# anthonyhu/tumblr-emotions

Measured on AMD Instinct MI355X. Metric: training samples/sec (224x224 img + 32-tok text, batch 256), higher is better.
Workload: dtype f32; 1 GPU; joint train step (fwd+bwd+all-reduce+Adam): Inception-v1 224x224x3 + 300-d embedding + LSTM-512, T=32, V=10000, 15 classes, batch 256 per GPU, reference freeze (<=Mixed_5b conv weights frozen, all BN betas trainable), dropout 0.8, BN train mode; global_batch=256, per_gpu_batch=256, parallelism=dp1, launch=eager

## Files before the change

### include/ds_kernels.h

```cpp
#ifndef DS_KERNELS_H
#define DS_KERNELS_H

#include <stddef.h>
#include <stdint.h>

#ifdef __cplusplus
extern "C" {
#endif

#define DS_OK 0
#define DS_ERR_ARG (-1)
#define DS_ERR_LAUNCH (-2)
#define DS_ERR_WORKSPACE (-3)

#define DS_DTYPE_F32 0
#define DS_DTYPE_BF16 1

#define DS_EPI_BIAS 1
#define DS_EPI_RELU 2
#define DS_EPI_ACCUM 4
#define DS_EPI_STATS 8
#define DS_EPI_MASK 16
#define DS_EPI_BNSUMS 32
#define DS_EPI_BN_RELU 64
// ... 203 lines not shown
int ds_conv_plan_enable_pool3(ds_conv_layer_plan *plan, uint8_t *argmax);
int ds_conv_plan_enable_bn_relu(ds_conv_layer_plan *plan);
int ds_conv_plan_finalize_tickets(const ds_conv_layer_plan *plan);
int ds_conv_prepare_weights(const ds_conv_layer_plan *plan, const float *w_hwio, void *w_prepared, float *wscale,
                            void *stream);
int ds_conv_run(const ds_conv_layer_plan *plan, const void *x, const void *w, float *z, const ds_conv_io *io, void *stream);

size_t ds_conv_wgrad_workspace(const ds_conv_desc *d);
int ds_conv_wgrad(const ds_conv_desc *d, const float *x, const float *dz, int32_t lddz, float *dw,
                  void *ws, size_t ws_bytes, void *stream);

int ds_bn_finalize(const float *stats, int32_t P, int64_t count, int32_t C, const float *beta, const float *pivot,
                   float eps, float decay, float *mean, float *rstd, float *shift, float *moving_mean,
                   float *moving_var, void *stream);

int ds_bn_finalize_centered(const float *stats, int32_t P, int64_t count, int32_t C, const float *beta, const float *pivot,
                            float eps, float decay, float *mean, float *rstd, float *shift, float *moving_mean,
                            float *moving_var, float *mean_c, float *shift_c, void *stream);
typedef struct ds_bn_finalize_job {
    const float *stats;
    int32_t P, C;
    int64_t count;
    const float *beta;
    const float *pivot;
    float *mean, *rstd, *shift;
    float *moving_mean, *moving_var;
} ds_bn_finalize_job;
int ds_bn_finalize_multi(const ds_bn_finalize_job *jobs, int32_t njobs, float eps, float decay, void *stream);

int ds_bn_finalize_apply_relu(const float *stats, int32_t P, int64_t count, int32_t C, const float *beta, const float *pivot,
                              float eps, float decay, float *mean, float *rstd, float *shift, float *moving_mean,
                              float *moving_var, const float *z, int64_t M, const struct ds_segments *dst, uint32_t *ticket,
                              void *stream);

typedef struct ds_segments {
    int32_t nseg;
    int32_t c_begin[4];
    int32_t c_end[4];
    int32_t ld[4];
    void *ptr[4];
    int32_t dtype[4];
    float *amax[4];
    const float *ptr2[4];
} ds_segments;
int ds_bn_apply_relu(const float *z, int64_t M, int32_t C, const float *rstd, const float *shift,
                     const ds_segments *dst, void *stream);
int ds_bn_apply_relu_z16(const void *z16, int64_t M, int32_t C, const float *rstd, const float *shift,
                         const ds_segments *dst, void *stream);
int ds_bn_infer_prepare(const float *beta, const float *moving_mean, const float *moving_var, float eps,
                        int32_t C, float *rstd, float *shift, void *stream);
typedef struct ds_bn_infer_job {
    const float *beta, *moving_mean, *moving_var;
    int32_t C;
    float *rstd, *shift;
} ds_bn_infer_job;
int ds_bn_infer_prepare_multi(const ds_bn_infer_job *jobs, int32_t njobs, float eps, void *stream);

int ds_bn_bwd_partials(int64_t M, int32_t C);
int ds_bn_bwd_reduce(const void *z, int32_t ldz, int32_t z_dtype, const ds_segments *dy, int64_t M, int32_t C,
                     const float *mean, const float *rstd, const float *shift, float *partials, void *stream);
int ds_bn_bwd_finalize(const float *partials, int32_t P, int64_t M, int32_t C, float *dbeta, float *coef,
                       void *stream);
typedef struct ds_bn_sum_segments {
    int32_t nseg;
    int32_t c_begin[4], c_end[4];
    int32_t P[4];
    int32_t kind[4];
    const float *s[4];
    const float *q[4];
    int32_t P2[4];
    const float *s2[4];
    const float *q2[4];
} ds_bn_sum_segments;
int ds_bn_bwd_finalize_segs(const ds_bn_sum_segments *sg, int64_t M, int32_t C, const float *beta, float *dbeta,
                            float *coef, void *stream);
int ds_bn_bwd_finalize_multi(const ds_bn_sum_segments *sg, int64_t M, int32_t C, const float *const *beta,
                             float *const *dbeta, float *coef, void *stream);
int ds_bn_bwd_finalize_apply(const ds_bn_sum_segments *sg, const float *beta, float *dbeta, const float *const *beta_v,
                             float *const *dbeta_v, float *coef, const float *z, int32_t ldz, const ds_segments *dy, int64_t M,
                             int32_t C, const float *mean, const float *rstd, const float *shift, void *dz, int32_t dz_dtype,
                             int32_t lddz, float *amax, uint32_t *ticket, void *stream);
int ds_bn_bwd_apply(const float *z, int32_t ldz, const ds_segments *dy, int64_t M, int32_t C, const float *mean,
                    const float *rstd, const float *shift, const float *coef, float *dz, float *amax, void *stream);
int ds_bn_infer_bwd_apply(const float *z, int32_t ldz, const ds_segments *dy, int64_t M, int32_t C, const float *rstd,
                          const float *shift, float *dz, void *stream);
int ds_bn_infer_bwd_partials(int64_t M, int32_t C);
int ds_bn_infer_bwd_apply_sums(const float *z, int32_t ldz, const ds_segments *dy, int64_t M, int32_t C, const float *rstd,
                               const float *shift, float *dz, float *partials, void *stream);
typedef struct ds_bn_sum_job {
    const float *partials;
    int32_t P, C;
    float *dbeta;
} ds_bn_sum_job;
int ds_bn_dbeta_reduce_multi(const ds_bn_sum_job *jobs, int32_t njobs, void *stream);
int ds_bn_bwd_apply_bf16(const float *z, int32_t ldz, const ds_segments *dy, int64_t M, int32_t C, const float *mean,
                         const float *rstd, const float *shift, const float *coef, void *dz16, int32_t lddz, float *amax,
                         void *stream);

int ds_bn_bwd_apply_z16(const void *z16, int32_t ldz, const ds_segments *dy, int64_t M, int32_t C, const float *mean,
                        const float *rstd, const float *shift, const float *coef, void *dz16, int32_t lddz, float *amax,
                        void *stream);

int ds_maxpool_fwd(const void *x, void *y, uint8_t *argmax, int32_t N, int32_t H, int32_t W, int32_t C,
                   int32_t k, int32_t stride, int32_t pad_t, int32_t pad_l, int32_t OH, int32_t OW,
                   int32_t act_dtype, void *stream);
int ds_maxpool_bn_relu_fwd(const float *z, const float *rstd, const float *shift, void *y, uint8_t *argmax,
                           int32_t N, int32_t H, int32_t W, int32_t C, int32_t k, int32_t stride, int32_t pad_t,
                           int32_t pad_l, int32_t OH, int32_t OW, int32_t y_dtype, float *amax, void *stream);
int ds_bn_pool_bwd_partials(int32_t N, int32_t OH, int32_t OW, int32_t C);
int ds_bn_pool_bwd_reduce(const float *z, const float *dpool, const uint8_t *argmax, int32_t N, int32_t H, int32_t W,
                          int32_t C, int32_t pad_t, int32_t pad_l, int32_t OH, int32_t OW, const float *mean,
                          const float *rstd, const float *shift, float *partials, void *stream);
int ds_bn_pool_bwd_apply(const float *z, const float *dpool, const uint8_t *argmax, int32_t N, int32_t H, int32_t W,
                         int32_t C, int32_t pad_t, int32_t pad_l, int32_t OH, int32_t OW, const float *mean,
                         const float *rstd, const float *shift, const float *coef, float *dz, void *stream);
int ds_bn_pool_infer_bwd_apply(const float *z, const float *dpool, const uint8_t *argmax, int32_t N, int32_t H, int32_t W,
                               int32_t C, int32_t pad_t, int32_t pad_l, int32_t OH, int32_t OW, const float *rstd,
                               const float *shift, float *dz, void *stream);
int ds_bn_pool_infer_bwd_apply_sums(const float *z, const float *dpool, const uint8_t *argmax, int32_t N, int32_t H, int32_t W,
                                    int32_t C, int32_t pad_t, int32_t pad_l, int32_t OH, int32_t OW, const float *rstd,
                                    const float *shift, float *dz, float *partials, void *stream);
int ds_maxpool_bwd(const float *dy, const uint8_t *argmax, float *dx, int32_t accumulate, int32_t N,
                   int32_t H, int32_t W, int32_t C, int32_t k, int32_t stride, int32_t pad_t, int32_t pad_l,
                   int32_t OH, int32_t OW, void *stream);

int ds_maxpool3_bwd_sums_partials(int32_t N, int32_t W, int32_t C);
int ds_maxpool3_bwd_sums(const float *dy, const uint8_t *argmax, float *dx, int32_t accumulate, const void *y,
                         int32_t y_dtype, int32_t N, int32_t H, int32_t W, int32_t C, float *partials, void *stream);

int ds_maxpool3_bwd_dy16(const void *dy16, const uint8_t *argmax, float *dx, int32_t accumulate, const void *y, int32_t y_dtype,
                         int32_t N, int32_t H, int32_t W, int32_t C, float *partials, void *stream);

int ds_avgpool_dropout_fwd(const float *x, int32_t N, int32_t HW, int32_t C, float keep, uint64_t seed,
                           const uint64_t *seed_dev, const float *mask_in, float *mask_out, float *out,
                           void *stream);
int ds_avgpool_dropout_bwd(const float *dout, const float *mask, int32_t N, int32_t HW, int32_t C,
                           float keep, float *dx, void *stream);

int ds_gather_rows(const float *table, const int64_t *ids, float *out, int32_t B, int32_t T, int32_t D,
                   int64_t table_rows, int32_t time_major, void *stream);

int ds_token_dot(const float *dx, const float *x, const int64_t *seq_len, float *out, int32_t B, int32_t T, int32_t D,
                 void *stream);

int ds_embedding_grad(const float *dx, const int64_t *ids, float *dtable, int32_t B, int32_t T, int32_t D,
                      int64_t table_rows, int32_t time_major, void *stream);

int ds_lstm_cell_fwd(float *gates, const float *rec_slabs, int32_t nslabs, int64_t slab_stride,
                     const float *c_prev, const float *h_prev, const int64_t *seq_len, int32_t t, int32_t B,
                     int32_t H, float forget_bias, float *c_out, float *h_out, void *stream);
int ds_lstm_cell_bwd(const float *acts, const float *c_t, const float *c_prev, const float *dh,
                     const float *dh_slabs, int32_t nslabs, int64_t slab_stride, const float *dc,
                     const int64_t *seq_len, int32_t t, int32_t B, int32_t H, float *dgates, float *dc_prev,
                     float *dh_carry, void *stream);

int ds_seq_sort_desc(const int64_t *seq_len, int32_t B, int32_t T, int32_t *perm, int64_t *len_sorted, void *stream);
int ds_permute_rows(const void *src, int64_t lds, void *dst, int64_t ldd, const int32_t *perm, int32_t rows, int32_t cols,
                    int32_t elem_bytes, int32_t gather, void *stream);
#define DS_LSTM_SKIP_MASKED 256
int ds_lstm_seq_supported(int32_t B, int32_t H);
size_t ds_lstm_seq_workspace(int32_t B, int32_t H);
int ds_lstm_seq_fwd(float *gates, const float *wh, int32_t ldw, float *h, float *c, const int64_t *seq_len, int32_t T,
                    int32_t B, int32_t H, float forget_bias, int32_t rows, void *ws, size_t ws_bytes, void *stream);
int ds_lstm_seq_bwd(const float *acts, const float *wh, int32_t ldw, const float *c, const float *dh_last,
                    int32_t ld_dh, const int64_t *seq_len, int32_t T, int32_t B, int32_t H, float *dgates, int32_t rows,
                    void *ws, size_t ws_bytes, void *stream);
int ds_lstm_seq_status(void *ws, int32_t B);
#ifdef DS_TUNING
int ds_debug_lstm_seq_set_profile(void *buf);
int ds_debug_lstm_seq_set_profile_bwd(void *buf);
#endif

int ds_softmax_ce(const float *logits, const int64_t *labels, int32_t B, int32_t C, float grad_scale,
                  const float *grad_scale_dev, float *loss, float *dlogits, void *stream);

int ds_adam_tf(float *theta, const float *g, float *m, float *v, int64_t n, int64_t n_wd, float wd,
               float grad_scale, float lr_t, const float *lr_t_dev, float beta1, float beta2, float eps,
               void *stream);

int ds_sumsq(const float *x, int64_t n, float *scratch, float *out, void *stream);
int ds_colsum(const float *x, int64_t M, int32_t C, int32_t ld, float *scratch, float *out, void *stream);
int ds_slab_epilogue(const float *slabs, int32_t splits, int64_t slab_stride, int32_t lds, int64_t M, int32_t N, float *out,
                     int32_t ldo, const float *bias, const float *mask, int32_t ldmask, int32_t flags, void *stream);
int ds_copy2d(const float *src, int32_t lds, float *dst, int32_t ldd, int64_t rows, int32_t cols,
              void *stream);
int ds_pad_channels(const float *src, int32_t cs, float *dst, int32_t cd, int64_t pixels, void *stream);
int ds_fill(float *dst, int64_t n, float value, void *stream);

typedef struct ds_preprocess_desc {
    int64_t offset;
    int32_t height, width;
    float scale_y, scale_x;
} ds_preprocess_desc;
int ds_preprocess_eval(const uint8_t *bytes, int64_t nbytes, const ds_preprocess_desc *desc, int32_t batch, const float *lut,
                       float *out, int32_t out_h, int32_t out_w, void *stream);

#define DS_PREPROCESS_FLIP 1u
#define DS_PREPROCESS_SATURATION_FIRST 2u
// ... 115 lines not shown
```

### tumblr_emotions_amd/_lib.py

```python
import ctypes as C
import os

_HERE = os.path.dirname(os.path.abspath(__file__))
LIB_PATH = os.environ.get("DS_LIB") or os.path.join(_HERE, "libds_kernels.so")

def tuning_env(name, default=None):
    return os.environ.get(name, default) if os.environ.get("DS_LIB") else default


DS_EPI_BIAS, DS_EPI_RELU, DS_EPI_ACCUM, DS_EPI_STATS, DS_EPI_MASK, DS_EPI_BNSUMS = 1, 2, 4, 8, 16, 32
DS_EPI_BN_RELU = 64
DS_DTYPE_F32, DS_DTYPE_BF16 = 0, 1
DS_FP8_E4M3, DS_FP8_E5M2 = 0, 1
DS_CONV_FWD, DS_CONV_DGRAD = 0, 1
DS_LSTM_SKIP_MASKED = 256
DS_ARITH_F32, DS_ARITH_BF16, DS_ARITH_FP8, DS_ARITH_F32X3 = 0, 1, 2, 3
DS_FAM_IGEMM, DS_FAM_WINO2, DS_FAM_WINO4, DS_FAM_STEM, DS_FAM_BF16D, DS_FAM_FP8D, DS_FAM_F32X3, DS_FAM_WINO4H, DS_FAM_STEM_POOL = range(9)
DS_FAM_STEM_DGRAD = 9
DS_PLAN_NO_WINO, DS_PLAN_NO_WINO4, DS_PLAN_NO_STEM_DIRECT, DS_PLAN_NO_BF16_DIRECT, DS_PLAN_ACT16, DS_PLAN_PACKED_RGB = 1, 2, 4, 8, 16, 32
DS_PLAN_FP8_EVERYWHERE, DS_PLAN_FP8_WIDE_RULE, DS_PLAN_NO_WINO4H, DS_PLAN_STEM_POOL = 64, 128, 256, 512
DS_PLAN_NO_SPLITK = 1024
DS_PREPROCESS_FLIP, DS_PREPROCESS_SATURATION_FIRST = 1, 2
DS_JPEG_UNSUPPORTED, DS_JPEG_MORE = 1, 2
DS_JPEG_444, DS_JPEG_422, DS_JPEG_420, DS_JPEG_GREY = 0, 1, 2, 3
# ... 112 lines not shown
_SS = C.POINTER(SumSegments)
_LP = C.POINTER(LayerPlanStruct)
_IO = C.POINTER(ConvIO)

SIGNATURES = {
    "ds_version": (C.c_int, []),
    "ds_last_error": (C.c_char_p, []),
    "ds_conv_igemm_partials": (C.c_int, [_CD]),
    "ds_conv_igemm_bnsums_supported": (C.c_int, [_CD]),
    "ds_conv_igemm_norm_supported": (C.c_int, [_CD]),
    "ds_conv_igemm_bnb_supported": (C.c_int, [_CD]),
    "ds_conv_igemm_pool3_supported": (C.c_int, [_CD]),
    "ds_conv_igemm_finalize_tickets": (C.c_int, [_CD]),
    "ds_conv_igemm": (C.c_int, [_CD, _P, _P, _P, _P, _P, _P, _P, _P]),
    "ds_weights_bf16_bytes": (C.c_size_t, [_i32, _i32, _i32, _i32]),
    "ds_weights_to_bf16": (C.c_int, [_P, _P, _i32, _i32, _i32, _i32, _P]),
    "ds_conv_bf16_supported": (C.c_int, [_CD]),
    "ds_conv_bf16_partials": (C.c_int, [_CD]),
    "ds_conv_bf16": (C.c_int, [_CD, _P, _P, _P, _P, _P, _P, _P]),
    "ds_weights_f32x3_bytes": (C.c_size_t, [_i32, _i32, _i32, _i32]),
    "ds_weights_to_f32x3": (C.c_int, [_P, _P, _i32, _i32, _i32, _i32, _P]),
    "ds_conv_f32x3_supported": (C.c_int, [_CD]),
    "ds_conv_f32x3_partials": (C.c_int, [_CD]),
    "ds_conv_f32x3": (C.c_int, [_CD, _P, _P, _P, _P, _P, _P, _P]),
    "ds_absmax": (C.c_int, [_P, _i64, _i32, _P, _P]),
    "ds_weights_fp8_bytes": (C.c_size_t, [_i32, _i32, _i32, _i32]),
    "ds_weights_to_fp8": (C.c_int, [_P, _P, _P, _i32, _i32, _i32, _i32, _P]),
    "ds_conv_fp8_supported": (C.c_int, [_CD]),
    "ds_conv_fp8_partials": (C.c_int, [_CD]),
    "ds_conv_fp8": (C.c_int, [_CD, _P, _P, _i32, _P, _P, _P, _P, _P, _P, _P]),
    "ds_conv_stem_partials": (C.c_int, [_i32, _i32, _i32]),
    "ds_conv_stem_bf16_partials": (C.c_int, [_i32, _i32, _i32]),
    "ds_conv_stem": (C.c_int, [_P, _P, _P, _P, _P, _i32, _i32, _i32, _i32, _i32, _i32, _P]),
    "ds_conv_stem_bf16": (C.c_int, [_P, _P, _P, _P, _P, _i32, _i32, _i32, _i32, _i32, _i32, _P]),
    "ds_conv_stem_pool_supported": (C.c_int, [_i32, _i32]),
    "ds_conv_stem_pool_partials": (C.c_int, [_i32, _i32, _i32]),
    "ds_conv_stem_pool": (C.c_int, [_P, _P, _P, _P, _P, _i32, _i32, _i32, _i32, _i32, _i32, _P]),
    "ds_conv_stem_pool_bf16": (C.c_int, [_P, _P, _P, _P, _P, _i32, _i32, _i32, _i32, _i32, _i32, _P]),
    "ds_conv_stem_dgrad_supported": (C.c_int, [_i32, _i32]),
    "ds_conv_stem_dgrad": (C.c_int, [_P, _P, _P, _i32, _i32, _i32, _i32, _i32, _P]),
    "ds_wino_transform_weights": (C.c_int, [_P, _P, _i32, _i32, _i32, _P]),
    "ds_conv_wino_partials": (C.c_int, [_i32, _i32, _i32]),
    "ds_conv_wino": (C.c_int, [_P, _P, _P, _P, _P, _P, _i32, _i32, _i32, _i32, _i32, _i32, _i32, _i32, _P]),
    "ds_conv_wino4_supported": (C.c_int, [_i32, _i32, _i32, _i32]),
    "ds_conv_wino4_prefer": (C.c_int, [_i32, _i32, _i32, _i32, _i32]),
    "ds_wino4_transform_weights": (C.c_int, [_P, _P, _i32, _i32, _i32, _P]),
    "ds_conv_wino4_partials": (C.c_int, [_i32, _i32, _i32]),
    "ds_conv_wino4_splitk_choose": (C.c_int, [_i32, _i32, _i32, _i32, _i32]),
    "ds_conv_wino4_splitk_partials": (C.c_int, [_i32, _i32, _i32]),
    "ds_conv_wino4_splitk_workspace": (C.c_size_t, [_i32, _i32, _i32, _i32, _i32]),
    "ds_conv_wino4_splitk": (C.c_int, [_P, _P, _P, _P, _P, _P, _i32, _i32, _i32, _i32, _i32, _i32, _i32, _i32, _i32, _i32, _P, C.c_size_t, _P]),
    "ds_conv_wino4": (C.c_int, [_P, _P, _P, _P, _P, _P, _i32, _i32, _i32, _i32, _i32, _i32, _i32, _i32, _P]),
    "ds_conv_wino4_bf16x2": (C.c_int, [_P, _P, _P, _P, _P, _P, _i32, _i32, _i32, _i32, _i32, _i32, _i32, _i32, _i32, _P]),
    "ds_conv_wino4_bf16x2_x16": (C.c_int, [_P, _P, _P, _P, _P, _P, _i32, _i32, _i32, _i32, _i32, _i32, _i32, _i32, _i32, _P]),
    "ds_wino4_transform_weights_bf16x2": (C.c_int, [_P, _P, _i32, _i32, _i32, _P]),
    "ds_conv_plan": (C.c_int, [_LP, _i32, _i32, C.c_uint32] + [_i32] * 10),
    "ds_conv_plan_set_flags": (C.c_int, [_LP, _i32]),
    "ds_conv_plan_enable_bnsums": (C.c_int, [_LP, _i32]),
    "ds_conv_plan_norm_supported": (C.c_int, [_LP]),
    "ds_conv_plan_bnb_supported": (C.c_int, [_LP]),
    "ds_conv_plan_enable_pool3": (C.c_int, [_LP, C.c_void_p]),
    "ds_conv_plan_enable_bn_relu": (C.c_int, [_LP]),
    "ds_conv_plan_finalize_tickets": (C.c_int, [_LP]),
    "ds_conv_prepare_weights": (C.c_int, [_LP, _P, _P, _P, _P]),
    "ds_conv_run": (C.c_int, [_LP, _P, _P, _P, _IO, _P]),
    "ds_conv_wgrad_workspace": (C.c_size_t, [_CD]),
    "ds_conv_wgrad": (C.c_int, [_CD, _P, _P, _i32, _P, _P, C.c_size_t, _P]),
    "ds_bn_finalize": (C.c_int, [_P, _i32, _i64, _i32, _P, _P, _f32, _f32, _P, _P, _P, _P, _P, _P]),
    "ds_bn_finalize_centered": (C.c_int, [_P, _i32, _i64, _i32, _P, _P, _f32, _f32, _P, _P, _P, _P, _P, _P, _P, _P]),
    "ds_bn_apply_relu": (C.c_int, [_P, _i64, _i32, _P, _P, _SG, _P]),
    "ds_bn_apply_relu_z16": (C.c_int, [_P, _i64, _i32, _P, _P, _SG, _P]),
    "ds_bn_bwd_apply_z16": (C.c_int, [_P, _i32, _SG, _i64, _i32, _P, _P, _P, _P, _P, _i32, _P, _P]),
    "ds_bn_infer_prepare": (C.c_int, [_P, _P, _P, _f32, _i32, _P, _P, _P]),
    "ds_bn_infer_prepare_multi": (C.c_int, [_P, _i32, _f32, _P]),
    "ds_bn_bwd_partials": (C.c_int, [_i64, _i32]),
    "ds_bn_bwd_reduce": (C.c_int, [_P, _i32, _i32, _SG, _i64, _i32, _P, _P, _P, _P, _P]),
    "ds_bn_bwd_finalize_segs": (C.c_int, [_SS, _i64, _i32, _P, _P, _P, _P]),
    "ds_bn_bwd_finalize": (C.c_int, [_P, _i32, _i64, _i32, _P, _P, _P]),
    "ds_bn_bwd_finalize_multi": (C.c_int, [_SS, _i64, _i32, _P, _P, _P, _P]),
    "ds_bn_finalize_multi": (C.c_int, [_P, _i32, _f32, _f32, _P]),
    "ds_bn_finalize_apply_relu": (C.c_int, [_P, _i32, _i64, _i32, _P, _P, _f32, _f32, _P, _P, _P, _P, _P, _P, _i64, _SG, _P, _P]),
    "ds_bn_bwd_finalize_apply": (C.c_int, [_SS, _P, _P, _P, _P, _P, _P, _i32, _SG, _i64, _i32, _P, _P, _P, _P, _i32, _i32, _P, _P, _P]),
    "ds_bn_bwd_apply": (C.c_int, [_P, _i32, _SG, _i64, _i32, _P, _P, _P, _P, _P, _P, _P]),
    "ds_bn_infer_bwd_apply": (C.c_int, [_P, _i32, _SG, _i64, _i32, _P, _P, _P, _P]),
    "ds_bn_infer_bwd_partials": (C.c_int, [_i64, _i32]),
    "ds_bn_infer_bwd_apply_sums": (C.c_int, [_P, _i32, _SG, _i64, _i32, _P, _P, _P, _P, _P]),
    "ds_bn_dbeta_reduce_multi": (C.c_int, [_P, _i32, _P]),
    "ds_bn_bwd_apply_bf16": (C.c_int, [_P, _i32, _SG, _i64, _i32, _P, _P, _P, _P, _P, _i32, _P, _P]),
    "ds_maxpool_fwd": (C.c_int, [_P, _P, _P] + [_i32] * 11 + [_P]),
    "ds_maxpool_bn_relu_fwd": (C.c_int, [_P, _P, _P, _P, _P] + [_i32] * 11 + [_P, _P]),
    "ds_bn_pool_bwd_partials": (C.c_int, [_i32, _i32, _i32, _i32]),
    "ds_bn_pool_bwd_reduce": (C.c_int, [_P, _P, _P] + [_i32] * 8 + [_P, _P, _P, _P, _P]),
    "ds_bn_pool_bwd_apply": (C.c_int, [_P, _P, _P] + [_i32] * 8 + [_P, _P, _P, _P, _P, _P]),
    "ds_bn_pool_infer_bwd_apply": (C.c_int, [_P, _P, _P] + [_i32] * 8 + [_P, _P, _P, _P]),
    "ds_bn_pool_infer_bwd_apply_sums": (C.c_int, [_P, _P, _P] + [_i32] * 8 + [_P, _P, _P, _P, _P]),
    "ds_maxpool_bwd": (C.c_int, [_P, _P, _P] + [_i32] * 11 + [_P]),
    "ds_maxpool3_bwd_sums_partials": (C.c_int, [_i32, _i32, _i32]),
    "ds_maxpool3_bwd_sums": (C.c_int, [_P, _P, _P, _i32, _P, _i32, _i32, _i32, _i32, _i32, _P, _P]),
    "ds_maxpool3_bwd_dy16": (C.c_int, [_P, _P, _P, _i32, _P, _i32, _i32, _i32, _i32, _i32, _P, _P]),
    "ds_avgpool_dropout_fwd": (C.c_int, [_P, _i32, _i32, _i32, _f32, _u64, _P, _P, _P, _P, _P]),
    "ds_avgpool_dropout_bwd": (C.c_int, [_P, _P, _i32, _i32, _i32, _f32, _P, _P]),
    "ds_gather_rows": (C.c_int, [_P, _P, _P, _i32, _i32, _i32, _i64, _i32, _P]),
    "ds_token_dot": (C.c_int, [_P, _P, _P, _P, _i32, _i32, _i32, _P]),
    "ds_embedding_grad": (C.c_int, [_P, _P, _P, _i32, _i32, _i32, _i64, _i32, _P]),
    "ds_lstm_cell_fwd": (C.c_int, [_P, _P, _i32, _i64, _P, _P, _P, _i32, _i32, _i32, _f32, _P, _P, _P]),
    "ds_lstm_cell_bwd": (C.c_int, [_P, _P, _P, _P, _P, _i32, _i64, _P, _P, _i32, _i32, _i32, _P, _P, _P, _P]),
    "ds_seq_sort_desc": (C.c_int, [_P, _i32, _i32, _P, _P, _P]),
    "ds_permute_rows": (C.c_int, [_P, _i64, _P, _i64, _P, _i32, _i32, _i32, _i32, _P]),
    "ds_lstm_seq_supported": (C.c_int, [_i32, _i32]),
    "ds_lstm_seq_workspace": (C.c_size_t, [_i32, _i32]),
    "ds_lstm_seq_fwd": (C.c_int, [_P, _P, _i32, _P, _P, _P, _i32, _i32, _i32, _f32, _i32, _P, C.c_size_t, _P]),
    "ds_lstm_seq_bwd": (C.c_int, [_P, _P, _i32, _P, _P, _i32, _P, _i32, _i32, _i32, _P, _i32, _P, C.c_size_t, _P]),
    "ds_lstm_seq_status": (C.c_int, [_P, _i32]),
    "ds_softmax_ce": (C.c_int, [_P, _P, _i32, _i32, _f32, _P, _P, _P, _P]),
    "ds_adam_tf": (C.c_int, [_P, _P, _P, _P, _i64, _i64, _f32, _f32, _f32, _P, _f32, _f32, _f32, _P]),
    "ds_sumsq": (C.c_int, [_P, _i64, _P, _P, _P]),
    "ds_colsum": (C.c_int, [_P, _i64, _i32, _i32, _P, _P, _P]),
    "ds_slab_epilogue": (C.c_int, [_P, _i32, _i64, _i32, _i64, _i32, _P, _i32, _P, _P, _i32, _i32, _P]),
    "ds_copy2d": (C.c_int, [_P, _i32, _P, _i32, _i64, _i32, _P]),
    "ds_pad_channels": (C.c_int, [_P, _i32, _P, _i32, _i64, _P]),
    "ds_fill": (C.c_int, [_P, _i64, _f32, _P]),
    "ds_preprocess_eval": (C.c_int, [_P, _i64, _P, _i32, _P, _P, _i32, _i32, _P]),
    "ds_preprocess_train": (C.c_int, [_P, _i64, _P, _i32, _P, _P, _i32, _i32, _P]),
    "ds_jpeg_probe": (C.c_int, [_P, _i64, C.POINTER(JpegInfo)]),
    "ds_jpeg_entropy_decode": (C.c_int, [_P, _i64, C.POINTER(JpegInfo), _P, _i64]),
    "ds_jpeg_reconstruct_host": (C.c_int, [_P, _i64, _P, _i32, _P, _i64]),
    "ds_jpeg_reconstruct": (C.c_int, [_P, _i64, _P, _i32, _P, _i64, _P, _i64, _P]),
    "ds_example_parse": (C.c_int, [_P, _i64, _P, _i32, C.POINTER(ExampleFields)]),
    "ds_jpeg_record_decode": (C.c_int, [_P, _i64, _P, _i32, C.POINTER(ExampleFields), C.POINTER(JpegInfo), _P, _i64,
                                        C.POINTER(_i32)]),
    "ds_jpeg_scan": (C.c_int, [_P, _i64, C.POINTER(JpegInfo), C.POINTER(JpegScanInfo), _P, _i64]),
    "ds_jpeg_record_scan": (C.c_int, [_P, _i64, _P, _i32, C.POINTER(ExampleFields), C.POINTER(JpegInfo), C.POINTER(JpegScanInfo),
                                      _P, _i64, C.POINTER(_i32)]),
    "ds_jpeg_restart_transcode": (C.c_int, [_P, _i64, _i32, _P, _i64, C.POINTER(_i64)]),
    "ds_jpeg_entropy_decode_segments_host": (C.c_int, [_P, _i64, _P, _i32, _P, _i64, _P, _i64, _P]),
    "ds_jpeg_entropy_decode_device": (C.c_int, [_P, _i64, _P, _i32, _P, _i64, _P, _i64, _P, _P]),
    "ds_ragged_gather": (C.c_int, [_P, _i64, _P, _i64, _P, _i32, _P, _i64, _P]),
    "ds_ragged_gather_host": (C.c_int, [_P, _i64, _P, _i64, _P, _i32, _P, _i64]),
}

_lib = None


DEBUG_SIGNATURES = {
    "ds_debug_conv_set_tile": (C.c_int, [C.c_int, C.c_int]),
    "ds_debug_conv_set_path": (C.c_int, [C.c_int]),
    "ds_debug_conv_set_wide": (C.c_int, [C.c_int]),
    "ds_debug_conv_wino_allow_ablation": (C.c_int, [C.c_int]),
    "ds_debug_conv_wino4_set_nb": (C.c_int, [C.c_int]),
    "ds_debug_conv_bf16_set_max_nb": (C.c_int, [C.c_int]),
    "ds_debug_lstm_seq_set_profile": (C.c_int, [_P]),
    "ds_debug_lstm_seq_set_profile_bwd": (C.c_int, [_P]),
}
TUNING_LIB_PATH = os.path.join(_HERE, "libds_kernels_tuning.so")
_tuning = None


def _bind(lib, table):
    for name, (res, args) in table.items():
        fn = getattr(lib, name)
        fn.restype = res
        fn.argtypes = args


def load_tuning():
    global _tuning
    if _tuning is None:
        if not os.path.exists(TUNING_LIB_PATH):
            raise RuntimeError("tumblr_emotions_amd: %s not found -- `make -C tumblr_emotions_amd/csrc` builds it" % TUNING_LIB_PATH)
        lib = C.CDLL(TUNING_LIB_PATH)
        _bind(lib, SIGNATURES)
        _bind(lib, DEBUG_SIGNATURES)
        _tuning = lib
    return _tuning


# ... 37 lines not shown
```

### tumblr_emotions_amd/csrc/bn.hip

```cpp
#include <stdlib.h>
#include "ds_common.h"

namespace {

struct SegDev {
    int nseg;
    int c_begin[4], c_end[4], ld[4];
    float *ptr[4];
    int dtype[4];
    float *amax[4];
    const float *ptr2[4];
};

SegDev to_dev(const ds_segments *s) {
    SegDev o;
    o.nseg = s->nseg;
    for (int i = 0; i < 4; ++i) {
        o.c_begin[i] = s->c_begin[i];
        o.c_end[i] = s->c_end[i];
        o.ld[i] = s->ld[i];
        o.ptr[i] = (float *)s->ptr[i];
        o.dtype[i] = s->dtype[i];
        o.amax[i] = s->amax[i];
        o.ptr2[i] = s->ptr2[i];
// ... 319 lines not shown
    s = wave_sum_f64(s);
    q = wave_sum_f64(q);
    if (lane == 0) {
        red[0][wave] = s;
        red[1][wave] = q;
    }
    __syncthreads();
    if (threadIdx.x == 0) {
        s = ((red[0][0] + red[0][1]) + red[0][2]) + red[0][3];
        q = ((red[1][0] + red[1][1]) + red[1][2]) + red[1][3];
        dbeta[c] = (float)s;
        if (coef) {
            coef[c] = (float)(s * inv_count);
            coef[C + c] = (float)(q * inv_count);
        }
    }
}

struct SumSegDev {
    int nseg;
    int c_begin[4], c_end[4], P[4], kind[4];
    const float *s[4], *q[4];
    int P2[4];
    const float *s2[4], *q2[4];
    const float *beta[4];
    float *dbeta[4];
};

template <bool COH = false>
__device__ __forceinline__ void bwd_finalize_segs_channel(const SumSegDev &sg, double inv_count, int C, float *coef, int c) {
    __shared__ double red[2][4];
    const int lane = threadIdx.x & 63, wave = threadIdx.x >> 6;
    int P = 0, kind = 0, P2 = 0;
    const float *sp = nullptr, *qp = nullptr, *beta = nullptr, *sp2 = nullptr, *qp2 = nullptr;
    float *dbeta = nullptr;
#pragma unroll
    for (int i = 0; i < 4; ++i)
        if (i < sg.nseg && c >= sg.c_begin[i] && c < sg.c_end[i]) {
            P = sg.P[i];
            kind = sg.kind[i];
            sp = sg.s[i] + (int64_t)(c - sg.c_begin[i]) * P;
            qp = sg.q[i] + (int64_t)(c - sg.c_begin[i]) * P;
            P2 = sg.P2[i];
            if (P2 > 0) {
                sp2 = sg.s2[i] + (int64_t)(c - sg.c_begin[i]) * P2;
                qp2 = sg.q2[i] + (int64_t)(c - sg.c_begin[i]) * P2;
            }
            beta = sg.beta[i] ? sg.beta[i] + (c - sg.c_begin[i]) : nullptr;
            dbeta = sg.dbeta[i] ? sg.dbeta[i] + (c - sg.c_begin[i]) : nullptr;
        }
    double s = 0.0, q = 0.0;
    for (int p = threadIdx.x; p < P; p += 256) {
        s += (double)sp[p];
        q += (double)qp[p];
    }
    for (int p = threadIdx.x; p < P2; p += 256) {
        s += (double)sp2[p];
        q += (double)qp2[p];
    }
    s = wave_sum_f64(s);
    q = wave_sum_f64(q);
    if (lane == 0) {
        red[0][wave] = s;
        red[1][wave] = q;
    }
    __syncthreads();
    if (threadIdx.x == 0) {
        s = ((red[0][0] + red[0][1]) + red[0][2]) + red[0][3];
        q = ((red[1][0] + red[1][1]) + red[1][2]) + red[1][3];
        if (kind == 1) q -= (double)*beta * s;
        if (dbeta) *dbeta = (float)s;
        st_res<COH>(coef + c, (float)(s * inv_count));
        st_res<COH>(coef + C + c, (float)(q * inv_count));
    }
}

__global__ __launch_bounds__(256) void bn_bwd_finalize_segs_kernel(SumSegDev sg, double inv_count, int C, float *coef) {
    bwd_finalize_segs_channel(sg, inv_count, C, coef, (int)blockIdx.x);
}

template <bool OUT16, bool COH = false, bool ADD2 = false, bool Z16 = false>
__device__ __forceinline__ void bwd_apply_body(int bid, const float *z, int ldz, const SegDev &dy, int64_t M, int C,
                                               const float *mean, const float *rstd, const float *shift,
                                               const float *coef, float *dz, float *amax, int drow, int lddz) {
    const int C4 = C >> 2;
    const int t0 = bid * 256 + threadIdx.x;
    const int row0 = t0 / C4, c = (t0 - row0 * C4) * 4;
    const float4 r4 = *reinterpret_cast<const float4 *>(rstd + c), s4 = *reinterpret_cast<const float4 *>(shift + c);
    const float4 m4 = *reinterpret_cast<const float4 *>(mean + c);
    const float4 k14 = ld_res4<COH>(coef + c), k24 = ld_res4<COH>(coef + C + c);
    const float rr[4] = {r4.x, r4.y, r4.z, r4.w}, ss[4] = {s4.x, s4.y, s4.z, s4.w}, mm[4] = {m4.x, m4.y, m4.z, m4.w};
    const float a1[4] = {k14.x, k14.y, k14.z, k14.w}, a2[4] = {k24.x, k24.y, k24.z, k24.w};
    int sgi = 0;
#pragma unroll
    for (int i = 1; i < 4; ++i)
        if (i < dy.nseg && c >= dy.c_begin[i] && c < dy.c_end[i]) sgi = i;
    const float *const dyp = dy.ptr[sgi] + (c - dy.c_begin[sgi]);
    const int64_t dyld = dy.ld[sgi];
    const float *const dyp2 = (ADD2 && dy.ptr2[sgi]) ? dy.ptr2[sgi] + (c - dy.c_begin[sgi]) : nullptr;
    float am = 0.f;
    constexpr int NR = DS_BN_ROWS;
    for (int64_t row = row0; row < M; row += NR * (int64_t)drow) {
        int64_t rws[NR];
        bool ok[NR];
#pragma unroll
        for (int u = 0; u < NR; ++u) {
            ok[u] = row + u * (int64_t)drow < M;
            rws[u] = ok[u] ? row + u * (int64_t)drow : row;
        }
        float4 zv[NR], dv[NR];
#pragma unroll
        for (int u = 0; u < NR; ++u) {
            if constexpr (Z16) zv[u] = ldz4<__bf16>(reinterpret_cast<const __bf16 *>(z) + rws[u] * ldz + c);
            else zv[u] = ds::ld_stream4(z + rws[u] * ldz + c);
            dv[u] = ds::ld_stream4(dyp + rws[u] * dyld);
        }
        if (ADD2 && dyp2) {
#pragma unroll
            for (int u = 0; u < NR; ++u) {
                const float4 e = ds::ld_stream4(dyp2 + rws[u] * dyld);
                dv[u].x += e.x; dv[u].y += e.y; dv[u].z += e.z; dv[u].w += e.w;
            }
        }
#pragma unroll
        for (int u = 0; u < NR; ++u) {
            if (u > 0 && !ok[u]) break;
            const float zz[4] = {zv[u].x, zv[u].y, zv[u].z, zv[u].w}, dd[4] = {dv[u].x, dv[u].y, dv[u].z, dv[u].w};
            float o[4];
#pragma unroll
            for (int j = 0; j < 4; ++j) o[j] = ds::bn_bwd_dz(zz[j], dd[j], rr[j], ss[j], mm[j], a1[j], a2[j]);
            if (OUT16) {
                const f32x4_t ov = {o[0], o[1], o[2], o[3]};
                *reinterpret_cast<bf16x4_t *>(reinterpret_cast<__bf16 *>(dz) + rws[u] * lddz + c) = __builtin_convertvector(ov, bf16x4_t);
            } else {
                *reinterpret_cast<float4 *>(dz + rws[u] * ldz + c) = make_float4(o[0], o[1], o[2], o[3]);
            }
            am = fmaxf(am, fmaxf(fmaxf(fabsf(o[0]), fabsf(o[1])), fmaxf(fabsf(o[2]), fabsf(o[3]))));
        }
    }
    if (amax) {
#pragma unroll
        for (int o = 32; o > 0; o >>= 1) am = fmaxf(am, __shfl_xor(am, o));
        if ((threadIdx.x & 63) == 0) ds::atomic_max_nonneg(amax, am);
    }
}

template <bool OUT16, bool ADD2 = false, bool Z16 = false>
__global__ __launch_bounds__(256) void bn_bwd_apply_kernel(const float *z, int ldz, SegDev dy, int64_t M, int C,
                                                           const float *mean, const float *rstd, const float *shift,
                                                           const float *coef, float *dz, float *amax, int drow, int lddz) {
    bwd_apply_body<OUT16, false, ADD2, Z16>((int)blockIdx.x, z, ldz, dy, M, C, mean, rstd, shift, coef, dz, amax, drow, lddz);
}

template <bool ADD2>
__global__ __launch_bounds__(256) void bn_infer_bwd_apply_kernel(const float *z, int ldz, SegDev dy, int64_t M, int C,
                                                                 const float *rstd, const float *shift, float *dz, int drow) {
    const int C4 = C >> 2;
    const int t0 = (int)blockIdx.x * 256 + threadIdx.x;
    const int row0 = t0 / C4, c = (t0 - row0 * C4) * 4;
    const float4 r4 = *reinterpret_cast<const float4 *>(rstd + c), s4 = *reinterpret_cast<const float4 *>(shift + c);
    const float rr[4] = {r4.x, r4.y, r4.z, r4.w}, ss[4] = {s4.x, s4.y, s4.z, s4.w};
    int sgi = 0;
#pragma unroll
    for (int i = 1; i < 4; ++i)
        if (i < dy.nseg && c >= dy.c_begin[i] && c < dy.c_end[i]) sgi = i;
    const float *const dyp = dy.ptr[sgi] + (c - dy.c_begin[sgi]);
    const int64_t dyld = dy.ld[sgi];
    const float *const dyp2 = (ADD2 && dy.ptr2[sgi]) ? dy.ptr2[sgi] + (c - dy.c_begin[sgi]) : nullptr;
    constexpr int NR = DS_BN_ROWS;
    for (int64_t row = row0; row < M; row += NR * (int64_t)drow) {
        int64_t rws[NR];
        bool ok[NR];
#pragma unroll
        for (int u = 0; u < NR; ++u) {
            ok[u] = row + u * (int64_t)drow < M;
            rws[u] = ok[u] ? row + u * (int64_t)drow : row;
        }
        float4 zv[NR], dv[NR];
#pragma unroll
        for (int u = 0; u < NR; ++u) {
            zv[u] = ds::ld_stream4(z + rws[u] * ldz + c);
            dv[u] = ds::ld_stream4(dyp + rws[u] * dyld);
        }
        if (ADD2 && dyp2) {
#pragma unroll
            for (int u = 0; u < NR; ++u) {
                const float4 e = ds::ld_stream4(dyp2 + rws[u] * dyld);
                dv[u].x += e.x; dv[u].y += e.y; dv[u].z += e.z; dv[u].w += e.w;
            }
        }
#pragma unroll
        for (int u = 0; u < NR; ++u) {
            if (u > 0 && !ok[u]) break;
            const float zz[4] = {zv[u].x, zv[u].y, zv[u].z, zv[u].w}, dd[4] = {dv[u].x, dv[u].y, dv[u].z, dv[u].w};
            f32x4_t o;
#pragma unroll
            for (int j = 0; j < 4; ++j) o[j] = __builtin_fmaf(zz[j], rr[j], ss[j]) > 0.f ? rr[j] * dd[j] : 0.f;
            __builtin_nontemporal_store(o, reinterpret_cast<f32x4_t *>(dz + rws[u] * ldz + c));
        }
    }
}

template <bool ADD2, bool WRITE>
__global__ __launch_bounds__(256) void bn_infer_bwd_apply_sums_kernel(const float *z, int ldz, SegDev dy, int64_t M, int C,
                                                                      const float *rstd, const float *shift, float *dz, int drow,
                                                                      float *partials) {
    __shared__ float sh[256][4];
    const int C4 = C >> 2;
    const int t0 = (int)blockIdx.x * 256 + threadIdx.x;
    const int row0 = t0 / C4, c = (t0 - row0 * C4) * 4;
    const float4 r4 = *reinterpret_cast<const float4 *>(rstd + c), s4 = *reinterpret_cast<const float4 *>(shift + c);
    const float rr[4] = {r4.x, r4.y, r4.z, r4.w}, ss[4] = {s4.x, s4.y, s4.z, s4.w};
    int sgi = 0;
#pragma unroll
    for (int i = 1; i < 4; ++i)
        if (i < dy.nseg && c >= dy.c_begin[i] && c < dy.c_end[i]) sgi = i;
    const float *const dyp = dy.ptr[sgi] + (c - dy.c_begin[sgi]);
    const int64_t dyld = dy.ld[sgi];
    const float *const dyp2 = (ADD2 && dy.ptr2[sgi]) ? dy.ptr2[sgi] + (c - dy.c_begin[sgi]) : nullptr;
    float sum[4] = {0.f, 0.f, 0.f, 0.f};
    constexpr int NR = DS_BN_ROWS;
    for (int64_t row = row0; row < M; row += NR * (int64_t)drow) {
        int64_t rws[NR];
        bool ok[NR];
#pragma unroll
        for (int u = 0; u < NR; ++u) {
            ok[u] = row + u * (int64_t)drow < M;
            rws[u] = ok[u] ? row + u * (int64_t)drow : row;
        }
        float4 zv[NR], dv[NR];
#pragma unroll
        for (int u = 0; u < NR; ++u) {
            zv[u] = ds::ld_stream4(z + rws[u] * ldz + c);
            dv[u] = ds::ld_stream4(dyp + rws[u] * dyld);
// ... 303 lines not shown
                   const float *const *beta_v, float *const *dbeta_v, float *coef, SumSegDev &d) {
    DS_REQUIRE(sg && coef && M > 0 && C > 0 && sg->nseg >= 1 && sg->nseg <= 4, "%s: bad argument", who);
    d.nseg = sg->nseg;
    int covered = 0;
    for (int i = 0; i < 4; ++i) {
        d.c_begin[i] = sg->c_begin[i]; d.c_end[i] = sg->c_end[i]; d.P[i] = sg->P[i]; d.kind[i] = sg->kind[i];
        d.s[i] = sg->s[i]; d.q[i] = sg->q[i];
        d.beta[i] = nullptr; d.dbeta[i] = nullptr;
        d.P2[i] = i < sg->nseg ? sg->P2[i] : 0; d.s2[i] = sg->s2[i]; d.q2[i] = sg->q2[i];
        if (i < sg->nseg) {
            DS_REQUIRE(sg->P2[i] >= 0 && (sg->P2[i] == 0 || (sg->s2[i] && sg->q2[i])), "%s: segment %d has a malformed second source", who, i);
            DS_REQUIRE(sg->s[i] && sg->q[i] && sg->P[i] > 0 && sg->c_end[i] > sg->c_begin[i] && (sg->kind[i] == 0 || sg->kind[i] == 1),
                       "%s: segment %d is malformed", who, i);
            d.beta[i] = beta_v ? beta_v[i] : (beta ? beta + sg->c_begin[i] : nullptr);
            d.dbeta[i] = dbeta_v ? dbeta_v[i] : (dbeta ? dbeta + sg->c_begin[i] : nullptr);
            DS_REQUIRE(sg->kind[i] == 0 || d.beta[i], "%s: DS_EPI_BNSUMS partials need beta", who);
            covered += sg->c_end[i] - sg->c_begin[i];
        }
    }
    DS_REQUIRE(covered == C, "%s: segments cover %d of %d channels", who, covered, C);
    return DS_OK;
}

int launch_finalize_segs(const char *who, const ds_bn_sum_segments *sg, int64_t M, int32_t C, const float *beta, float *dbeta,
                         const float *const *beta_v, float *const *dbeta_v, float *coef, void *stream) {
    SumSegDev d;
    if (int e = build_sum_segs(who, sg, M, C, beta, dbeta, beta_v, dbeta_v, coef, d)) return e;
    hipLaunchKernelGGL(bn_bwd_finalize_segs_kernel, dim3(C), dim3(256), 0, (hipStream_t)stream, d, 1.0 / (double)M, C, coef);
    return ds::check_launch(who);
}
}

extern "C" int ds_bn_bwd_finalize_segs(const ds_bn_sum_segments *sg, int64_t M, int32_t C, const float *beta,
                                       float *dbeta, float *coef, void *stream) {
    return launch_finalize_segs("ds_bn_bwd_finalize_segs", sg, M, C, beta, dbeta, nullptr, nullptr, coef, stream);
}

extern "C" int ds_bn_bwd_finalize_multi(const ds_bn_sum_segments *sg, int64_t M, int32_t C, const float *const *beta,
                                        float *const *dbeta, float *coef, void *stream) {
    DS_REQUIRE(beta, "ds_bn_bwd_finalize_multi: the segments' beta vectors are required");
    return launch_finalize_segs("ds_bn_bwd_finalize_multi", sg, M, C, nullptr, nullptr, beta, dbeta, coef, stream);
}

extern "C" int ds_bn_bwd_finalize_apply(const ds_bn_sum_segments *sg, const float *beta, float *dbeta, const float *const *beta_v,
                                        float *const *dbeta_v, float *coef, const float *z, int32_t ldz, const ds_segments *dy,
                                        int64_t M, int32_t C, const float *mean, const float *rstd, const float *shift, void *dz,
                                        int32_t dz_dtype, int32_t lddz, float *amax, uint32_t *ticket, void *stream) {
    const bool out16 = dz_dtype == DS_DTYPE_BF16;
    DS_REQUIRE(z && mean && rstd && shift && coef && dz && ticket && M > 0 && C > 0 && C % 4 == 0 && ldz >= C && ldz % 4 == 0 &&
                   (((uintptr_t)z) & 15) == 0 && (dz_dtype == DS_DTYPE_F32 || out16) &&
                   (((uintptr_t)dz) & (out16 ? 7 : 15)) == 0 && (!out16 || (lddz >= C && lddz % 4 == 0)),
               "ds_bn_bwd_finalize_apply: bad argument (see ds_bn_bwd_apply / ds_bn_bwd_apply_bf16)");
    if (int e = check_segments(dy, C, "ds_bn_bwd_finalize_apply")) return e;
    DS_REQUIRE(!has_second_addend(dy), "ds_bn_bwd_finalize_apply: no second addend (use ds_bn_bwd_finalize_segs + ds_bn_bwd_apply)");
    BwdFinApplyArgs a;
    if (int e = build_sum_segs("ds_bn_bwd_finalize_apply", sg, M, C, beta, dbeta, beta_v, dbeta_v, coef, a.sg)) return e;
    a.inv_count = 1.0 / (double)M; a.C = C; a.coef = coef;
    a.z = z; a.ldz = ldz; a.dy = to_dev(dy); a.M = M;
    a.mean = mean; a.rstd = rstd; a.shift = shift;
    a.dz = reinterpret_cast<float *>(dz); a.amax = amax; a.lddz = out16 ? lddz : ldz;
    a.ticket = ticket;
    const int grid = column_grid(M, C / 4, &a.drow);
    if (out16) hipLaunchKernelGGL(bn_bwd_finalize_apply_kernel<true>, dim3(C + grid), dim3(256), 0, (hipStream_t)stream, a);
    else hipLaunchKernelGGL(bn_bwd_finalize_apply_kernel<false>, dim3(C + grid), dim3(256), 0, (hipStream_t)stream, a);
    return ds::check_launch("ds_bn_bwd_finalize_apply");
}

extern "C" int ds_bn_bwd_apply(const float *z, int32_t ldz, const ds_segments *dy, int64_t M, int32_t C, const float *mean,
                               const float *rstd, const float *shift, const float *coef, float *dz, float *amax,
                               void *stream) {
    DS_REQUIRE(z && mean && rstd && shift && coef && dz && M > 0 && C > 0 && C % 4 == 0 && ldz >= C && ldz % 4 == 0 &&
                   ((((uintptr_t)z) | ((uintptr_t)dz)) & 15) == 0,
               "ds_bn_bwd_apply: bad argument (need C %% 4 == 0, ldz >= C, ldz %% 4 == 0, 16-byte aligned z / dz)");
    if (int e = check_segments(dy, C, "ds_bn_bwd_apply")) return e;
    int drow;
    const int grid = column_grid(M, C / 4, &drow);
    if (has_second_addend(dy))
        hipLaunchKernelGGL((bn_bwd_apply_kernel<false, true>), dim3(grid), dim3(256), 0, (hipStream_t)stream, z, ldz, to_dev(dy), M, C, mean,
                           rstd, shift, coef, dz, amax, drow, ldz);
    else
        hipLaunchKernelGGL(bn_bwd_apply_kernel<false>, dim3(grid), dim3(256), 0, (hipStream_t)stream, z, ldz, to_dev(dy), M, C, mean, rstd,
                           shift, coef, dz, amax, drow, ldz);
    return ds::check_launch("ds_bn_bwd_apply");
}

extern "C" int ds_bn_bwd_apply_z16(const void *z16, int32_t ldz, const ds_segments *dy, int64_t M, int32_t C, const float *mean,
                                   const float *rstd, const float *shift, const float *coef, void *dz16, int32_t lddz,
                                   float *amax, void *stream) {
    DS_REQUIRE(z16 && mean && rstd && shift && coef && dz16 && M > 0 && C > 0 && C % 4 == 0 && ldz >= C && ldz % 4 == 0 &&
                   lddz >= C && lddz % 4 == 0 && (((uintptr_t)z16) & 7) == 0 && (((uintptr_t)dz16) & 7) == 0 && z16 != dz16,
               "ds_bn_bwd_apply_z16: bad argument (need C %% 4 == 0, ldz / lddz >= C and %% 4 == 0, 8-byte aligned z / dz, dz != z)");
    if (int e = check_segments(dy, C, "ds_bn_bwd_apply_z16")) return e;
    int drow;
    const int grid = column_grid(M, C / 4, &drow);
    const float *zf = reinterpret_cast<const float *>(z16);
    if (has_second_addend(dy))
        hipLaunchKernelGGL((bn_bwd_apply_kernel<true, true, true>), dim3(grid), dim3(256), 0, (hipStream_t)stream, zf, ldz, to_dev(dy), M, C,
                           mean, rstd, shift, coef, reinterpret_cast<float *>(dz16), amax, drow, lddz);
    else
        hipLaunchKernelGGL((bn_bwd_apply_kernel<true, false, true>), dim3(grid), dim3(256), 0, (hipStream_t)stream, zf, ldz, to_dev(dy), M, C,
                           mean, rstd, shift, coef, reinterpret_cast<float *>(dz16), amax, drow, lddz);
    return ds::check_launch("ds_bn_bwd_apply_z16");
}

extern "C" int ds_bn_bwd_apply_bf16(const float *z, int32_t ldz, const ds_segments *dy, int64_t M, int32_t C, const float *mean,
                                    const float *rstd, const float *shift, const float *coef, void *dz16, int32_t lddz,
                                    float *amax, void *stream) {
    DS_REQUIRE(z && mean && rstd && shift && coef && dz16 && M > 0 && C > 0 && C % 4 == 0 && ldz >= C && ldz % 4 == 0 &&
                   lddz >= C && lddz % 4 == 0 && (((uintptr_t)z) & 15) == 0 && (((uintptr_t)dz16) & 7) == 0,
               "ds_bn_bwd_apply_bf16: bad argument (need C %% 4 == 0, ldz / lddz >= C and %% 4 == 0, aligned z / dz)");
    if (int e = check_segments(dy, C, "ds_bn_bwd_apply_bf16")) return e;
    int drow;
    const int grid = column_grid(M, C / 4, &drow);
    if (has_second_addend(dy))
        hipLaunchKernelGGL((bn_bwd_apply_kernel<true, true>), dim3(grid), dim3(256), 0, (hipStream_t)stream, z, ldz, to_dev(dy), M, C, mean,
                           rstd, shift, coef, reinterpret_cast<float *>(dz16), amax, drow, lddz);
    else
        hipLaunchKernelGGL(bn_bwd_apply_kernel<true>, dim3(grid), dim3(256), 0, (hipStream_t)stream, z, ldz, to_dev(dy), M, C, mean,
                           rstd, shift, coef, reinterpret_cast<float *>(dz16), amax, drow, lddz);
    return ds::check_launch("ds_bn_bwd_apply_bf16");
}

extern "C" int ds_bn_infer_bwd_apply(const float *z, int32_t ldz, const ds_segments *dy, int64_t M, int32_t C, const float *rstd,
                                     const float *shift, float *dz, void *stream) {
    DS_REQUIRE(z && rstd && shift && dz && M > 0 && C > 0 && C % 4 == 0 && ldz >= C && ldz % 4 == 0 &&
                   ((((uintptr_t)z) | ((uintptr_t)dz) | ((uintptr_t)rstd) | ((uintptr_t)shift)) & 15) == 0,
               "ds_bn_infer_bwd_apply: bad argument (need C %% 4 == 0, ldz >= C, ldz %% 4 == 0, 16-byte aligned z / dz / rstd / shift)");
    if (int e = check_segments(dy, C, "ds_bn_infer_bwd_apply")) return e;
    int drow;
    const int grid = column_grid(M, C / 4, &drow);
    if (has_second_addend(dy))
        hipLaunchKernelGGL(bn_infer_bwd_apply_kernel<true>, dim3(grid), dim3(256), 0, (hipStream_t)stream, z, ldz, to_dev(dy), M, C, rstd,
                           shift, dz, drow);
    else
        hipLaunchKernelGGL(bn_infer_bwd_apply_kernel<false>, dim3(grid), dim3(256), 0, (hipStream_t)stream, z, ldz, to_dev(dy), M, C, rstd,
                           shift, dz, drow);
    return ds::check_launch("ds_bn_infer_bwd_apply");
}

extern "C" int ds_bn_infer_bwd_partials(int64_t M, int32_t C) {
    if (M <= 0 || C <= 0 || C % 4) return 0;
    int drow;
    return column_grid(M, C / 4, &drow);
}

extern "C" int ds_bn_infer_bwd_apply_sums(const float *z, int32_t ldz, const ds_segments *dy, int64_t M, int32_t C,
                                          const float *rstd, const float *shift, float *dz, float *partials, void *stream) {
    DS_REQUIRE(z && rstd && shift && partials && M > 0 && C > 0 && C % 4 == 0 && ldz >= C && ldz % 4 == 0 &&
                   ((((uintptr_t)z) | ((uintptr_t)dz) | ((uintptr_t)rstd) | ((uintptr_t)shift)) & 15) == 0 &&
                   (((uintptr_t)partials) & 3) == 0,
               "ds_bn_infer_bwd_apply_sums: bad argument (need C %% 4 == 0, ldz >= C, ldz %% 4 == 0, 16-byte aligned z / dz / rstd / "
               "shift, partials)");
    if (int e = check_segments(dy, C, "ds_bn_infer_bwd_apply_sums")) return e;
    int drow;
    const int grid = column_grid(M, C / 4, &drow);
    const bool add2 = has_second_addend(dy);
    hipStream_t st = (hipStream_t)stream;
    if (add2 && dz)
        hipLaunchKernelGGL((bn_infer_bwd_apply_sums_kernel<true, true>), dim3(grid), dim3(256), 0, st, z, ldz, to_dev(dy), M, C, rstd, shift,
                           dz, drow, partials);
    else if (add2)
        hipLaunchKernelGGL((bn_infer_bwd_apply_sums_kernel<true, false>), dim3(grid), dim3(256), 0, st, z, ldz, to_dev(dy), M, C, rstd, shift,
                           dz, drow, partials);
    else if (dz)
        hipLaunchKernelGGL((bn_infer_bwd_apply_sums_kernel<false, true>), dim3(grid), dim3(256), 0, st, z, ldz, to_dev(dy), M, C, rstd, shift,
                           dz, drow, partials);
// ... 26 lines not shown
```

### tumblr_emotions_amd/csrc/pool.hip

```cpp
#include <type_traits>
#include "ds_common.h"

namespace {

typedef __bf16 bf16x4 __attribute__((ext_vector_type(4)));
typedef float f32x4v __attribute__((ext_vector_type(4)));
template <typename T>
__device__ __forceinline__ float4 ld4(const T *p);
template <>
__device__ __forceinline__ float4 ld4<float>(const float *p) { return *reinterpret_cast<const float4 *>(p); }
template <>
__device__ __forceinline__ float4 ld4<__bf16>(const __bf16 *p) {
    const f32x4v v = __builtin_convertvector(*reinterpret_cast<const bf16x4 *>(p), f32x4v);
    return make_float4(v[0], v[1], v[2], v[3]);
}
__device__ __forceinline__ void st4(float *p, float a, float b, float c, float d) {
    *reinterpret_cast<float4 *>(p) = make_float4(a, b, c, d);
}
__device__ __forceinline__ void st4(__bf16 *p, float a, float b, float c, float d) {
    const f32x4v v = {a, b, c, d};
    *reinterpret_cast<bf16x4 *>(p) = __builtin_convertvector(v, bf16x4);
}

template <typename TI, typename TO>
// ... 605 lines not shown
                    const float g = (zz[j] * rr[j] + ss[j] > 0.f) ? pg.g[y][x][j] : 0.f;
                    sg[j] += g;
                    sx[j] += g * ((zz[j] - mm[j]) * rr[j]);
                }
            }
        }
    }
#pragma unroll
    for (int j = 0; j < 4; ++j) {
        sh[threadIdx.x][j] = sg[j];
        sh[threadIdx.x][4 + j] = sx[j];
    }
    __syncthreads();
    if (threadIdx.x < C4) {
        const int cg = threadIdx.x;
        int t0 = (int)(((int64_t)cg - (int64_t)blockIdx.x * 256) % C4);
        if (t0 < 0) t0 += C4;
        float a[8] = {0, 0, 0, 0, 0, 0, 0, 0};
        for (int t = t0; t < 256; t += C4)
#pragma unroll
            for (int j = 0; j < 8; ++j) a[j] += sh[t][j];
        const int P = gridDim.x;
#pragma unroll
        for (int j = 0; j < 4; ++j) {
            partials[(int64_t)(cg * 4 + j) * P + blockIdx.x] = a[j];
            partials[((int64_t)C + cg * 4 + j) * P + blockIdx.x] = a[4 + j];
        }
    }
}

__global__ __launch_bounds__(256) void bn_pool_bwd_apply_kernel(const float *z, const float *dpool, const uint8_t *am,
                                                                int N, int H, int W, int C, int pad_t, int pad_l, int OH,
                                                                int OW, const float *mean, const float *rstd,
                                                                const float *shift, const float *coef, float *dz) {
    const int C4 = C >> 2;
    const int PH = OH + 1, PW = OW + 1;
    const int64_t total = (int64_t)N * PH * PW * C4;
    for (int64_t i = (int64_t)blockIdx.x * 256 + threadIdx.x; i < total; i += (int64_t)gridDim.x * 256) {
        const int c = (int)(i % C4) * 4;
        int64_t r = i / C4;
        const int q = (int)(r % PW) - 1;
        r /= PW;
        const int p = (int)(r % PH) - 1;
        const int n = (int)(r / PH);
        const PatchGrad pg = patch_grad(dpool, am, n, p, q, c, C, OH, OW);
        const float4 r4 = *reinterpret_cast<const float4 *>(rstd + c);
        const float4 s4 = *reinterpret_cast<const float4 *>(shift + c);
        const float4 m4 = *reinterpret_cast<const float4 *>(mean + c);
        const float4 k1 = *reinterpret_cast<const float4 *>(coef + c);
        const float4 k2 = *reinterpret_cast<const float4 *>(coef + C + c);
        const float rr[4] = {r4.x, r4.y, r4.z, r4.w}, ss[4] = {s4.x, s4.y, s4.z, s4.w}, mm[4] = {m4.x, m4.y, m4.z, m4.w};
        const float a1[4] = {k1.x, k1.y, k1.z, k1.w}, a2[4] = {k2.x, k2.y, k2.z, k2.w};
        float4 zv[2][2];
        bool ok[2][2];
        int64_t offs[2][2];
#pragma unroll
        for (int y = 0; y < 2; ++y)
#pragma unroll
            for (int x = 0; x < 2; ++x) {
                const int ih = 2 * p - pad_t + 1 + y, iw = 2 * q - pad_l + 1 + x;
                ok[y][x] = (unsigned)ih < (unsigned)H && (unsigned)iw < (unsigned)W;
                offs[y][x] = (((int64_t)n * H + ih) * W + iw) * C + c;
                zv[y][x] = make_float4(0.f, 0.f, 0.f, 0.f);
                if (ok[y][x]) zv[y][x] = ds::ld_stream4(z + offs[y][x]);
            }
#pragma unroll
        for (int y = 0; y < 2; ++y)
#pragma unroll
            for (int x = 0; x < 2; ++x) {
                if (!ok[y][x]) continue;
                const float zz[4] = {zv[y][x].x, zv[y][x].y, zv[y][x].z, zv[y][x].w};
                float o[4];
#pragma unroll
                for (int j = 0; j < 4; ++j) {
                    const float g = (zz[j] * rr[j] + ss[j] > 0.f) ? pg.g[y][x][j] : 0.f;
                    const float xhat = (zz[j] - mm[j]) * rr[j];
                    o[j] = rr[j] * (g - a1[j] - xhat * a2[j]);
                }
                *reinterpret_cast<float4 *>(dz + offs[y][x]) = make_float4(o[0], o[1], o[2], o[3]);
            }
    }
}

__global__ __launch_bounds__(256) void bn_pool_infer_bwd_apply_kernel(const float *z, const float *dpool, const uint8_t *am,
                                                                      int N, int H, int W, int C, int pad_t, int pad_l, int OH,
                                                                      int OW, const float *rstd, const float *shift, float *dz) {
    const int C4 = C >> 2;
    const int PH = OH + 1, PW = OW + 1;
    const int64_t total = (int64_t)N * PH * PW * C4;
    for (int64_t i = (int64_t)blockIdx.x * 256 + threadIdx.x; i < total; i += (int64_t)gridDim.x * 256) {
        const int c = (int)(i % C4) * 4;
        int64_t r = i / C4;
        const int q = (int)(r % PW) - 1;
        r /= PW;
        const int p = (int)(r % PH) - 1;
        const int n = (int)(r / PH);
        const PatchGrad pg = patch_grad(dpool, am, n, p, q, c, C, OH, OW);
        const float4 r4 = *reinterpret_cast<const float4 *>(rstd + c);
        const float4 s4 = *reinterpret_cast<const float4 *>(shift + c);
        const float rr[4] = {r4.x, r4.y, r4.z, r4.w}, ss[4] = {s4.x, s4.y, s4.z, s4.w};
        float4 zv[2][2];
        bool ok[2][2];
        int64_t offs[2][2];
#pragma unroll
        for (int y = 0; y < 2; ++y)
#pragma unroll
            for (int x = 0; x < 2; ++x) {
                const int ih = 2 * p - pad_t + 1 + y, iw = 2 * q - pad_l + 1 + x;
                ok[y][x] = (unsigned)ih < (unsigned)H && (unsigned)iw < (unsigned)W;
                offs[y][x] = (((int64_t)n * H + ih) * W + iw) * C + c;
                zv[y][x] = make_float4(0.f, 0.f, 0.f, 0.f);
                if (ok[y][x]) zv[y][x] = ds::ld_stream4(z + offs[y][x]);
            }
#pragma unroll
        for (int y = 0; y < 2; ++y)
#pragma unroll
            for (int x = 0; x < 2; ++x) {
                if (!ok[y][x]) continue;
                const float zz[4] = {zv[y][x].x, zv[y][x].y, zv[y][x].z, zv[y][x].w};
                ds::f32x4_nt o;
#pragma unroll
                for (int j = 0; j < 4; ++j) o[j] = __builtin_fmaf(zz[j], rr[j], ss[j]) > 0.f ? rr[j] * pg.g[y][x][j] : 0.f;
                __builtin_nontemporal_store(o, reinterpret_cast<ds::f32x4_nt *>(dz + offs[y][x]));
            }
    }
}

template <bool WRITE>
__global__ __launch_bounds__(256) void bn_pool_infer_bwd_apply_sums_kernel(const float *z, const float *dpool, const uint8_t *am,
                                                                           int N, int H, int W, int C, int pad_t, int pad_l, int OH,
                                                                           int OW, const float *rstd, const float *shift, float *dz,
                                                                           float *partials) {
    __shared__ float sh[256][4];
    const int C4 = C >> 2;
    const int PH = OH + 1, PW = OW + 1;
    const int64_t total = (int64_t)N * PH * PW * C4;
    const int64_t first = (int64_t)blockIdx.x * 256 + threadIdx.x;
    const int c = (int)(first % C4) * 4;
    const float4 r4 = *reinterpret_cast<const float4 *>(rstd + c);
    const float4 s4 = *reinterpret_cast<const float4 *>(shift + c);
    const float rr[4] = {r4.x, r4.y, r4.z, r4.w}, ss[4] = {s4.x, s4.y, s4.z, s4.w};
    float sum[4] = {0.f, 0.f, 0.f, 0.f};
    for (int64_t i = first; i < total; i += (int64_t)gridDim.x * 256) {
        int64_t r = i / C4;
        const int q = (int)(r % PW) - 1;
        r /= PW;
        const int p = (int)(r % PH) - 1;
        const int n = (int)(r / PH);
        const PatchGrad pg = patch_grad(dpool, am, n, p, q, c, C, OH, OW);
        float4 zv[2][2];
        bool ok[2][2];
        int64_t offs[2][2];
#pragma unroll
        for (int y = 0; y < 2; ++y)
#pragma unroll
            for (int x = 0; x < 2; ++x) {
                const int ih = 2 * p - pad_t + 1 + y, iw = 2 * q - pad_l + 1 + x;
                ok[y][x] = (unsigned)ih < (unsigned)H && (unsigned)iw < (unsigned)W;
                offs[y][x] = (((int64_t)n * H + ih) * W + iw) * C + c;
                zv[y][x] = make_float4(0.f, 0.f, 0.f, 0.f);
                if (ok[y][x]) zv[y][x] = ds::ld_stream4(z + offs[y][x]);
            }
#pragma unroll
        for (int y = 0; y < 2; ++y)
#pragma unroll
            for (int x = 0; x < 2; ++x) {
// ... 132 lines not shown
        hipLaunchKernelGGL((maxpool3s1_bwd_sums_kernel<__bf16, __bf16>), dim3(sh.P * sh.chunks), dim3(256), shmem, (hipStream_t)stream, dy, argmax, dx,
                           accumulate, (const __bf16 *)y, N, H, W, C, partials, sh.upb, sh.CW, sh.chunks);
    else
        hipLaunchKernelGGL((maxpool3s1_bwd_sums_kernel<float, __bf16>), dim3(sh.P * sh.chunks), dim3(256), shmem, (hipStream_t)stream, dy, argmax, dx,
                           accumulate, (const float *)y, N, H, W, C, partials, sh.upb, sh.CW, sh.chunks);
    return ds::check_launch("ds_maxpool3_bwd_dy16");
}

extern "C" int ds_maxpool3_bwd_sums(const float *dy, const uint8_t *argmax, float *dx, int32_t accumulate, const void *y,
                                    int32_t y_dtype, int32_t N, int32_t H, int32_t W, int32_t C, float *partials,
                                    void *stream) {
    DS_REQUIRE(dy && argmax && dx && y && partials && N > 0 && H > 0 && W > 0 && C > 0 && C % 4 == 0 && C <= 1024,
               "ds_maxpool3_bwd_sums: bad argument (C %% 4 == 0, C <= 1024)");
    DS_REQUIRE(y_dtype == DS_DTYPE_F32 || y_dtype == DS_DTYPE_BF16, "ds_maxpool3_bwd_sums: y_dtype must be DS_DTYPE_F32 or DS_DTYPE_BF16");
    DS_REQUIRE((int64_t)N * H * W * C < (1ll << 40), "ds_maxpool3_bwd_sums: tensor too large");
    const PoolSumsShape sh = pool_sums_shape(N, W, C);
    const size_t shmem = (size_t)sh.RG * sh.CW * 8 * sizeof(float);
    if (y_dtype == DS_DTYPE_BF16)
        hipLaunchKernelGGL((maxpool3s1_bwd_sums_kernel<__bf16, float>), dim3(sh.P * sh.chunks), dim3(256), shmem, (hipStream_t)stream, dy, argmax, dx,
                           accumulate, (const __bf16 *)y, N, H, W, C, partials, sh.upb, sh.CW, sh.chunks);
    else
        hipLaunchKernelGGL((maxpool3s1_bwd_sums_kernel<float, float>), dim3(sh.P * sh.chunks), dim3(256), shmem, (hipStream_t)stream, dy, argmax, dx,
                           accumulate, (const float *)y, N, H, W, C, partials, sh.upb, sh.CW, sh.chunks);
    return ds::check_launch("ds_maxpool3_bwd_sums");
}

extern "C" int ds_avgpool_dropout_fwd(const float *x, int32_t N, int32_t HW, int32_t C, float keep, uint64_t seed,
                                      const uint64_t *seed_dev, const float *mask_in, float *mask_out, float *out,
                                      void *stream) {
    DS_REQUIRE(x && out && C % 4 == 0 && N > 0 && HW > 0 && keep > 0.f, "ds_avgpool_dropout_fwd: bad argument");
    hipLaunchKernelGGL(avgpool_dropout_fwd_kernel, dim3(N), dim3(256), 0, (hipStream_t)stream, x, N, HW, C, keep, seed,
                       seed_dev, mask_in, mask_out, out);
    return ds::check_launch("ds_avgpool_dropout_fwd");
}

extern "C" int ds_avgpool_dropout_bwd(const float *dout, const float *mask, int32_t N, int32_t HW, int32_t C,
                                      float keep, float *dx, void *stream) {
    DS_REQUIRE(dout && dx && C % 4 == 0 && keep > 0.f, "ds_avgpool_dropout_bwd: bad argument");
    const float scale = (keep >= 1.f ? 1.f : 1.f / keep) / (float)HW;
    const int64_t total = (int64_t)N * HW * (C / 4);
    hipLaunchKernelGGL(avgpool_dropout_bwd_kernel, dim3(ds::stream_grid(total, 256)), dim3(256), 0,
                       (hipStream_t)stream, dout, keep >= 1.f ? nullptr : mask, N, HW, C, scale, dx);
    return ds::check_launch("ds_avgpool_dropout_bwd");
}

namespace {
int pool_bwd_grid(int N, int OH, int OW, int C) {
    const int C4 = C / 4;
    const int64_t total = (int64_t)N * (OH + 1) * (OW + 1) * C4;
    int g = ds::stream_grid(total, 256 * 4);
    int a = 256, b = C4;
    while (b) { const int t = a % b; a = b; b = t; }
    const int step = C4 / a;
    g = (g + step - 1) / step * step;
    return g;
}
}

extern "C" int ds_bn_pool_bwd_partials(int32_t N, int32_t OH, int32_t OW, int32_t C) { return pool_bwd_grid(N, OH, OW, C); }

extern "C" int ds_bn_pool_bwd_reduce(const float *z, const float *dpool, const uint8_t *argmax, int32_t N, int32_t H,
                                     int32_t W, int32_t C, int32_t pad_t, int32_t pad_l, int32_t OH, int32_t OW,
                                     const float *mean, const float *rstd, const float *shift, float *partials,
                                     void *stream) {
    DS_REQUIRE(z && dpool && argmax && mean && rstd && shift && partials && C % 4 == 0 && C <= 1024 && H <= 2 * OH &&
                   W <= 2 * OW,
               "ds_bn_pool_bwd_reduce: bad argument (3x3 stride-2 SAME pools, C %% 4 == 0, C <= 1024)");
    hipLaunchKernelGGL(bn_pool_bwd_reduce_kernel, dim3(pool_bwd_grid(N, OH, OW, C)), dim3(256), 0, (hipStream_t)stream, z,
                       dpool, argmax, N, H, W, C, pad_t, pad_l, OH, OW, mean, rstd, shift, partials);
    return ds::check_launch("ds_bn_pool_bwd_reduce");
}

extern "C" int ds_bn_pool_bwd_apply(const float *z, const float *dpool, const uint8_t *argmax, int32_t N, int32_t H,
                                    int32_t W, int32_t C, int32_t pad_t, int32_t pad_l, int32_t OH, int32_t OW,
                                    const float *mean, const float *rstd, const float *shift, const float *coef,
                                    float *dz, void *stream) {
    DS_REQUIRE(z && dpool && argmax && mean && rstd && shift && coef && dz && C % 4 == 0 && H <= 2 * OH && W <= 2 * OW,
               "ds_bn_pool_bwd_apply: bad argument (3x3 stride-2 SAME pools, C %% 4 == 0)");
    hipLaunchKernelGGL(bn_pool_bwd_apply_kernel, dim3(pool_bwd_grid(N, OH, OW, C)), dim3(256), 0, (hipStream_t)stream, z,
                       dpool, argmax, N, H, W, C, pad_t, pad_l, OH, OW, mean, rstd, shift, coef, dz);
    return ds::check_launch("ds_bn_pool_bwd_apply");
}

extern "C" int ds_bn_pool_infer_bwd_apply(const float *z, const float *dpool, const uint8_t *argmax, int32_t N, int32_t H,
                                          int32_t W, int32_t C, int32_t pad_t, int32_t pad_l, int32_t OH, int32_t OW,
                                          const float *rstd, const float *shift, float *dz, void *stream) {
    DS_REQUIRE(z && dpool && argmax && rstd && shift && dz && N > 0 && H > 0 && W > 0 && OH > 0 && OW > 0 && C > 0 && C % 4 == 0 &&
                   H <= 2 * OH && W <= 2 * OW && pad_t >= 0 && pad_t <= 1 && pad_l >= 0 && pad_l <= 1 &&
                   ((((uintptr_t)z) | ((uintptr_t)dz) | ((uintptr_t)dpool) | ((uintptr_t)rstd) | ((uintptr_t)shift)) & 15) == 0,
               "ds_bn_pool_infer_bwd_apply: bad argument (3x3 stride-2 SAME pools, C %% 4 == 0, 16-byte aligned tensors)");
    hipLaunchKernelGGL(bn_pool_infer_bwd_apply_kernel, dim3(pool_bwd_grid(N, OH, OW, C)), dim3(256), 0, (hipStream_t)stream, z,
                       dpool, argmax, N, H, W, C, pad_t, pad_l, OH, OW, rstd, shift, dz);
    return ds::check_launch("ds_bn_pool_infer_bwd_apply");
}

extern "C" int ds_bn_pool_infer_bwd_apply_sums(const float *z, const float *dpool, const uint8_t *argmax, int32_t N, int32_t H,
                                               int32_t W, int32_t C, int32_t pad_t, int32_t pad_l, int32_t OH, int32_t OW,
                                               const float *rstd, const float *shift, float *dz, float *partials, void *stream) {
    DS_REQUIRE(z && dpool && argmax && rstd && shift && partials && N > 0 && H > 0 && W > 0 && OH > 0 && OW > 0 && C > 0 &&
                   C % 4 == 0 && H <= 2 * OH && W <= 2 * OW && pad_t >= 0 && pad_t <= 1 && pad_l >= 0 && pad_l <= 1 &&
                   ((((uintptr_t)z) | ((uintptr_t)dz) | ((uintptr_t)dpool) | ((uintptr_t)rstd) | ((uintptr_t)shift)) & 15) == 0 &&
                   (((uintptr_t)partials) & 3) == 0,
               "ds_bn_pool_infer_bwd_apply_sums: bad argument (3x3 stride-2 SAME pools, C %% 4 == 0, 16-byte aligned tensors, partials)");
    const int grid = pool_bwd_grid(N, OH, OW, C);
    if (dz)
        hipLaunchKernelGGL(bn_pool_infer_bwd_apply_sums_kernel<true>, dim3(grid), dim3(256), 0, (hipStream_t)stream, z, dpool, argmax, N,
                           H, W, C, pad_t, pad_l, OH, OW, rstd, shift, dz, partials);
    else
        hipLaunchKernelGGL(bn_pool_infer_bwd_apply_sums_kernel<false>, dim3(grid), dim3(256), 0, (hipStream_t)stream, z, dpool, argmax, N,
                           H, W, C, pad_t, pad_l, OH, OW, rstd, shift, dz, partials);
    return ds::check_launch("ds_bn_pool_infer_bwd_apply_sums");
}
```

### tumblr_emotions_amd/engine_image.py

```python
import contextlib
import ctypes as C
import os
from collections import namedtuple

import torch

from . import _lib, ops
from .ops import WgradPlan, gemm_plan, make_segments, same_pad, DS_EPI_BIAS, DS_EPI_STATS

BN_EPS = 0.001
BN_DECAY = 0.9997
WEIGHT_DECAY = 0.00004

TOPOLOGY = [
    ("conv", "Conv2d_1a_7x7", 7, 2, 64),
    ("maxpool", "MaxPool_2a_3x3", 3, 2),
    ("conv", "Conv2d_2b_1x1", 1, 1, 64),
    ("conv", "Conv2d_2c_3x3", 3, 1, 192),
    ("maxpool", "MaxPool_3a_3x3", 3, 2),
    ("mixed", "Mixed_3b", 64, (96, 128), (16, 32), 32),
    ("mixed", "Mixed_3c", 128, (128, 192), (32, 96), 64),
    ("maxpool", "MaxPool_4a_3x3", 3, 2),
    ("mixed", "Mixed_4b", 192, (96, 208), (16, 48), 64),
    ("mixed", "Mixed_4c", 160, (112, 224), (24, 64), 64),
# ... 78 lines not shown
        fp8 = eng.dtype == "fp8" and not self.fold and k in (1, 3) and self.stride == 1
        if fp8:
            self.amax = torch.zeros(2, ops.AMAX_FLOATS, device=dev)
            self.dz_amax = eng.new_amax()
        self.u_version = -1
        self._fused = None
        eng._fused_key = None
        eng.need_stats(self.fwd.partials * 2 * cout)
        self.bwd_P = ops.bn_bwd_partials(self.M, cout)
        eng.need_bwd_partials(self.bwd_P * 2 * cout)
        self.pool_P = ops.bn_pool_bwd_partials(B, self.OH, self.OW, cout)
        eng.need_bwd_partials(self.pool_P * 2 * cout)
        self.dgrad = None
        self.z16 = False
        self.wgrad = None
        self.dy_parts = None
        self._dz_amax_live = False
        self.dx_sums = None
        self.bnb = False
        self.dx_y = None
        self._sum_segs = None
        self.fz_job = None
        self._fz_part = None
        self._fz_segs = None
        if self.trainable:
            if self.fold:
                self.wgrad = WgradPlan(B, self.H, self.W, 7 * 4, 4, 7, 1, self.stride, cout, cout, fold_cin=4)
            else:
                self.wgrad = WgradPlan(B, self.H, self.W, cin, 0, k, k, self.stride, cout, cout)
            eng.need_ws(self.wgrad.ws_bytes)

    def use_concat_slice(self, zview, ld, rstd, shift, mean=None):
        self.z, self.ldz, self.rstd, self.shift, self.skip_apply = zview, ld, rstd, shift, True
        if mean is not None:
            self.mean = mean
        self.fwd.d.ldz = ld

    @property
    def zmean(self):
        return self.mean_c if self.z16 else self.mean

    @property
    def zshift(self):
        return self.shift_c if self.z16 else self.shift

    def plan_finalize(self):
        eng = self.eng
        self.fin = None
        n = self.fwd.finalize_tickets() if eng.fuse_finalize else 0
        if n > 0:
            self.fin_tickets = torch.zeros(n, dtype=torch.int32, device=eng.device)
            f = _lib.BnFinalizeInLaunch()
            f.ticket, f.eps, f.decay = self.fin_tickets.data_ptr(), BN_EPS, BN_DECAY
            self.fin = f

    def bind(self):
        st = self.eng.store
        self.w_ptr = _vp(st.ptr(self.key + "/weights"))
        self.beta = st.view(self.key + "/BatchNorm/beta")
        self.mm = st.view(self.key + "/BatchNorm/moving_mean")
        self.mv = st.view(self.key + "/BatchNorm/moving_variance")
        self.mean.copy_(self.mm)
        eng = self.eng
        self.stats_buf, self.bwdp_buf, self.ws_buf = eng.stats_set[self.slot], eng.bwdp_set[self.slot], eng.ws_set[self.slot]
        for plan in (self.fwd, self.dgrad):
            if plan is not None and plan.ws_bytes:
                plan.set_workspace(eng.cws_set[self.slot])
        self.plan_finalize()
        if self.fin is not None:
            f = self.fin
            f.beta, f.mean, f.rstd, f.shift = self.beta.data_ptr(), self.mean.data_ptr(), self.rstd.data_ptr(), self.shift.data_ptr()
        self.gw_ptr = _vp(st.grad_ptr(self.key + "/weights")) if self.trainable else None
        self.gbeta = st.grad_view(self.key + "/BatchNorm/beta") if self.eng.trainable_bn_beta else None

    def set_dy_parts(self, parts):
        self.dy_parts = parts
        self.dy_segs = make_segments(parts)
        self.part_segs = [make_segments([(0, c1 - c0, ptr, ld)]) for (c0, c1, ptr, ld) in parts]
        self.part_sums = [None] * len(parts)
        self.part_sums2 = [None] * len(parts)
        self.dy2 = False
        self.part_pool = [None] * len(parts)
        self._sum_segs = None

    def sums_from(self, part, src, src2=None):
        self.part_sums[part], self.part_sums2[part] = src, src2
        self._sum_segs = None

    def sums_from_pool(self, part, pool, off):
        self.part_pool[part] = (pool, off)
        self._sum_segs = None

    def emit_dx_sums(self, y):
        eng = self.eng
        if not eng.bwd_sums or self.dgrad is None:
            return None
        P = self.dgrad.enable_bnsums(self.dgrad.d.ldz)
        if not P:
            return None
        self.dgrad.d.mask_dtype = ops.act_dtype(y)
        self.dx_sums = torch.empty(2 * self.cin * P, device=eng.device)
        self.dx_y = y
        return SumSource(self.dx_sums, P, 0, self.cin)

    def _sum_plan(self):
        if self._sum_segs is None:
            sg = ops.SumSegments()
            sg.nseg = len(self.dy_parts)
            self._reduce_jobs = []
            self._sync_views = []
            scratch, P0 = self.bwdp_buf.data_ptr(), self.bwd_P
            for i, (c0, c1, _, _) in enumerate(self.dy_parts):
                sg.c_begin[i], sg.c_end[i] = c0, c1
                src = self.part_sums[i]
                if src is not None:
                    sg.P[i], sg.kind[i] = src.P, 1
                    sg.s[i], sg.q[i] = src.ptrs()
                    self._sync_views += src.views(c1 - c0)
                    src2 = self.part_sums2[i]
                    if src2 is not None:
                        sg.P2[i] = src2.P
                        sg.s2[i], sg.q2[i] = src2.ptrs()
                        self._sync_views += src2.views(c1 - c0)
                    continue
                n, dst = c1 - c0, _vp(scratch)
                if self.part_pool[i] is None:
                    job, P = FullReduce(i, c0, n, dst), P0
                else:
                    job = self._pool_reduce(*self.part_pool[i], c0, n, dst)
                    P = ops.bn_bwd_partials(job.M, n)
                sg.P[i], sg.kind[i] = P, 0
                sg.s[i], sg.q[i] = scratch, scratch + 4 * n * P
                o0 = (scratch - self.bwdp_buf.data_ptr()) // 4
                self._sync_views.append(self.bwdp_buf[o0:o0 + 2 * n * P])
                self._reduce_jobs.append(job)
                scratch += 4 * 2 * n * P
            self._sum_segs = sg
        return self._sum_segs

    def _pool_reduce(self, pool, off, c0, n, dst):
        eng = self.eng
        if pool.raw:
            stat = (_vp(self.mean.data_ptr() + 4 * c0), _vp(self.rstd.data_ptr() + 4 * c0), _vp(self.shift.data_ptr() + 4 * c0))
        else:
            stat = (_vp(self.beta.data_ptr() + 4 * c0), ops._p(eng.ones), ops._p(eng.zeros))
        return PoolReduce(make_segments([(0, n, pool.dout.data_ptr() + 4 * off, pool.C)]), pool.B * pool.H * pool.W, n,
                          _vp(pool.out.data_ptr() + pool.out.element_size() * off), pool.C, *stat, dst, ops.act_dtype(pool.out))

    def _run_reduce_jobs(self):
        for job in self._reduce_jobs:
            if isinstance(job, PoolReduce):
                ops.bn_bwd_reduce(job.y, job.segs, job.M, job.n, job.mean, job.rstd, job.shift, job.dst, ldz=job.ldy,
                                  z_dtype=job.y_dtype)
                continue
            off = 4 * job.c0
            ops.bn_bwd_reduce(_vp(self.z.data_ptr() + self.z.element_size() * job.c0), self.part_segs[job.part], self.M, job.n,
                              _vp(self.zmean.data_ptr() + off), _vp(self.rstd.data_ptr() + off), _vp(self.zshift.data_ptr() + off),
                              job.dst, ldz=self.ldz, z_dtype=ops.act_dtype(self.z))

    def _bn_bwd_sums(self):
        sg = self._sum_plan()
        self._run_reduce_jobs()
        self._finalize(lambda count, gbeta: ops.bn_bwd_finalize_segs(sg, count, self.cout, self.beta, gbeta, self.coef),
                       self._sync_views)

    def _finalize_plain(self, P):
# ... 165 lines not shown
            self.wgrad.run(x_ptr, ops._p(self.z), self.gw_ptr, ops._p(self.ws_buf), eng.ws_bytes)
        if need_dx:
            self._run_dgrad(dx_ptr)

    def backward_infer(self, dx_ptr, pool=None, apply=True, run_dgrad=True):
        if apply:
            if pool is not None:
                ops.bn_pool_infer_bwd_apply(self.z, pool.dout, pool.argmax, self.B, self.OH, self.OW, self.cout, self.rstd,
                                            self.shift, self.z)
            else:
                ops.bn_infer_bwd_apply(self.z, self.dy_segs, self.M, self.cout, self.rstd, self.shift, self.z, ldz=self.ldz)
        self._dz_amax_live = False
        if run_dgrad:
            self._run_dgrad(dx_ptr)

    def frozen_partials(self, pool=None):
        if self._fz_part is None:
            if self.pool_inside:
                P = ops.bn_infer_bwd_partials(self.z.shape[0], self.cout)
            elif pool is not None:
                P = ops.bn_pool_bwd_partials(self.B, self.OH, self.OW, self.cout)
            else:
                P = ops.bn_infer_bwd_partials(self.M, self.cout)
            self._fz_part = torch.empty(self.cout * P, device=self.eng.device)
            self.fz_job = (self._fz_part.data_ptr(), P)
        return self._fz_part

    def backward_frozen(self, x_ptr=None, ldx=0, dx_ptr=None, need_dx=True, pool=None, apply=True):
        if self.gbeta is None and not need_dx and not self.trainable:
            return
        want_dz = need_dx or self.trainable
        dz = self.z if want_dz else None
        if apply and self.gbeta is None:
            if want_dz:
                self.backward_infer(None, pool, run_dgrad=False)
        elif apply:
            part = self.frozen_partials(pool)
            if self.pool_inside:
                assert pool is not None and not want_dz
                if self._fz_segs is None:
                    self._fz_segs = make_segments([(0, self.cout, pool.dout.data_ptr(), self.cout)])
                ops.bn_infer_bwd_apply_sums(self.z, self._fz_segs, self.z.shape[0], self.cout, self.rstd, self.shift, None, part)
            elif pool is not None:
                ops.bn_pool_infer_bwd_apply_sums(self.z, pool.dout, pool.argmax, self.B, self.OH, self.OW, self.cout, self.rstd,
                                                 self.shift, dz, part)
            else:
                ops.bn_infer_bwd_apply_sums(self.z, self.dy_segs, self.M, self.cout, self.rstd, self.shift, dz, part, ldz=self.ldz)
        self._dz_amax_live = False
        if self.trainable:
            self._run_wgrad(x_ptr, ldx)
        if need_dx:
            self._run_dgrad(dx_ptr)

    def _run_wgrad(self, x_ptr, ldx):
        eng = self.eng
        self.wgrad.d.ldx = ldx
        if eng.wgrad_stream is not None:
            ev = torch.cuda.Event()
            ev.record(torch.cuda.current_stream())
            eng.wgrad_stream.wait_event(ev)
            with torch.cuda.stream(eng.wgrad_stream):
                self.wgrad.run(x_ptr, ops._p(self.z), self.gw_ptr, ops._p(eng.ws_set[3]), eng.ws_bytes)
            eng.wgrad_pending = True
        else:
            self.wgrad.run(x_ptr, ops._p(self.z), self.gw_ptr, ops._p(self.ws_buf), eng.ws_bytes)

    def _run_dgrad(self, dx_ptr, use16=False):
        sums = ops._p(self.dx_sums) if self.dx_sums is not None else None
        y = ops._p(self.dx_y) if self.dx_sums is not None else None
        if self.eng.infer_bwd:
            sums = y = None
        am = None
        if self.dgrad.family == ops.DS_FAM_FP8D:
            am = self.dz_amax if self._dz_amax_live else self.amax[1]
            if not self._dz_amax_live:
                ops.absmax(self.z, self.M * self.cout, am)
        if use16:
            self.dgrad.d.x_dtype = ops.DS_DTYPE_BF16
            self.dgrad.run(ops._p(self.dz16), self.w_ptr, dx_ptr, mask=y, stats=sums, x_amax=ops._p(am))
            return
        self.dgrad.d.x_dtype = ops.DS_DTYPE_F32
        self.dgrad.run(ops._p(self.z), self.w_ptr, dx_ptr, mask=y, stats=sums, x_amax=ops._p(am))

    def backward(self, x_ptr=None, ldx=0, dx_ptr=None, need_dx=True):
        eng = self.eng
        M, Cc = self.M, self.cout
        dy_segs = self.dy_segs
        if self.gbeta is None and not need_dx and not self.trainable:
            return
        from_parts = any(ps is not None for ps in self.part_sums) or any(pp is not None for pp in self.part_pool)
        track = self.dgrad is not None and self.dgrad.family == ops.DS_FAM_FP8D
        dz = self.z if self.dz16 is None else self.dz16
        if eng.fuse_fin_apply and not eng.sync_bn and (need_dx or self.trainable) and not self.bnb and not self.dy2 and not self.z16:
            if from_parts:
                sg = self._sum_plan()
                self._run_reduce_jobs()
            else:
                ops.bn_bwd_reduce(self.z, dy_segs, M, Cc, self.zmean, self.rstd, self.zshift, self.bwdp_buf, ldz=self.ldz)
                if self._plain_segs is None:
                    sg = ops.SumSegments()
                    sg.nseg = 1
                    sg.c_begin[0], sg.c_end[0], sg.P[0], sg.kind[0] = 0, Cc, self.bwd_P, 0
                    sg.s[0], sg.q[0] = self.bwdp_buf.data_ptr(), self.bwdp_buf.data_ptr() + 4 * Cc * self.bwd_P
                    self._plain_segs = sg
                sg = self._plain_segs
            ops.bn_bwd_finalize_apply(sg, M, Cc, self.beta, self.gbeta, self.coef, self.z, dy_segs, self.mean, self.rstd,
                                      self.shift, dz, self.fa_ticket[2:4], amax=self.dz_amax if track else None, ldz=self.ldz)
        else:
            if from_parts:
                self._bn_bwd_sums()
            else:
                ops.bn_bwd_reduce(self.z, dy_segs, M, Cc, self.zmean, self.rstd, self.zshift, self.bwdp_buf, ldz=self.ldz)
                self._finalize_plain(self.bwd_P)
            if not (need_dx or self.trainable):
                return
            if self.bnb:
                self._run_dgrad(dx_ptr)
                return
            ops.bn_bwd_apply(self.z, dy_segs, M, Cc, self.zmean, self.rstd, self.zshift, self.coef, dz,
                             amax=self.dz_amax if track else None, ldz=self.ldz)
        self._dz_amax_live = track
        if self.trainable:
            self._run_wgrad(x_ptr, ldx)
        if need_dx:
            self._run_dgrad(dx_ptr, use16=self.dz16 is not None)


class Stage:
    name = ""
    out = None
    dout = None
    next = None
    zcat = False
    rs_cat = None
    raw = False
    out_amax = None
    fused_into_pool = False
    track_amax = True


class InputStage(Stage):
    def __init__(self, eng, size):
        self.eng, self.H, self.W, self.C = eng, size, size, 4
        self.name = "input"

    def alloc(self, B):
        self.out = torch.zeros(B, self.H, self.W, 4, device=self.eng.device)
        self.dout = None


class ConvStage(Stage):
    def __init__(self, eng, name, prev, k, stride, cout, trainable, beta_bucket):
        self.eng, self.name, self.prev = eng, name, prev
        fold = isinstance(prev, InputStage)
        cin = 3 if fold else prev.C
        self.layer = ConvBN(eng, [("InceptionV1/" + name, 0, cout)], k, stride, cin, cout, prev.H, prev.W, trainable,
                            beta_bucket, fold=fold)
        self.H, self.W, self.C = self.layer.OH, self.layer.OW, cout
        self.layers = [self.layer]
        self.pool = None

    def alloc(self, B):
        eng, dev = self.eng, self.eng.device
        self.layer.pool_inside = self.pool_inside_wanted()
        self.layer.alloc(B)
        self.out16 = self.eng.act16 and not self.layer.fold
        self.out = torch.empty(B, self.H, self.W, self.C, device=dev, dtype=torch.bfloat16 if self.out16 else torch.float32)
        self.dout = torch.empty(B, self.H, self.W, self.C, device=dev)
        self.out_amax = self.eng.new_amax()
        self.segs = make_segments([(0, self.C, self.out.data_ptr(), self.C, ops.act_dtype(self.out),
                                    ops._p(self.out_amax))])
        self.layer.set_dy_parts([(0, self.C, self.dout.data_ptr(), self.C)])
        self.norm_in = None
        if self.prev.raw:
            assert self.layer.fwd.norm_supported()
            self.norm_in = self.prev.rs
            self.layer.fwd.d.norm_rstd, self.layer.fwd.d.norm_shift = self.norm_in[0].data_ptr(), self.norm_in[1].data_ptr()
        if not self.layer.fold:
            self.layer.make_dgrad(self.prev.C)
            if isinstance(self.prev, ConvStage) and not self.prev.layer.fold:
                src = self.layer.emit_dx_sums(self.prev.out)
                if src is not None:
                    self.prev.layer.sums_from(0, src)
            if isinstance(self.prev, PoolStage) and self.prev.zmax is not None and eng.stem_sums_from_dgrad:
                stem = self.prev.prev.layer
                src = self.layer.emit_dx_sums(self.prev.out)
                if src is not None:
                    if self.prev.raw:
                        self.layer.dgrad.d.mask_rstd, self.layer.dgrad.d.mask_shift = stem.rstd.data_ptr(), stem.shift.data_ptr()
                    stem.sums_from(0, src)

    def pool_inside_wanted(self):
        eng, nxt = self.eng, self.next
        return bool(self.layer.fold and eng.stem_pool and eng.stem_direct and eng.fuse_bn_pool and not eng.input_grad
                    and not eng.mul3 and not self.layer.trainable
                    and isinstance(nxt, PoolStage) and nxt.k == 3 and nxt.stride == 2)

    def forward(self):
        self.layer.forward(ops._p(self.prev.out), self.prev.C, None if self.pool_applies_bn() else self.segs,
                           ops.act_dtype(self.prev.out), self.prev.out_amax)

    def pool_applies_bn(self):
        return self.fused_into_pool and not (self.eng.fused_infer and not self.layer.fold)

    def backward(self, need_dx):
        need_dx = need_dx and (not self.layer.fold or self.eng.input_grad)
        dx = ops._p(self.prev.dout) if need_dx else None
        if self.eng.frozen_step:
            self.layer.backward_frozen(ops._p(self.prev.out), self.prev.C, dx, need_dx,
                                       self.pool if (self.fused_into_pool and self.pool.stride == 2) else None)
            return
        if self.eng.infer_bwd:
            self.layer.backward_infer(dx, self.pool if (self.fused_into_pool and self.pool.stride == 2) else None)
            return
        if self.fused_into_pool and self.pool.stride == 2:
            self.layer.backward_pooled(self.pool, ops._p(self.prev.out), self.prev.C, dx, need_dx)
        else:
            self.layer.backward(ops._p(self.prev.out), self.prev.C, dx, need_dx)


class PoolStage(Stage):
    def __init__(self, eng, name, prev, k, stride):
        self.eng, self.name, self.prev, self.k, self.stride = eng, name, prev, k, stride
        self.H, _ = same_pad(prev.H, k, stride)
        self.W, _ = same_pad(prev.W, k, stride)
        self.C = prev.C
        self.layers = []

    def alloc(self, B):
        dev = self.eng.device
        self.B = B
        p = self.prev
        o16 = p.out.dtype == torch.bfloat16 or (self.eng.act16 and isinstance(p, ConvStage) and self.k == 3)
        inside = isinstance(p, ConvStage) and p.layer.pool_inside
        self.raw, self.rs, self.zmax = False, None, None
        if inside:
            self.zmax = p.layer.z.view(B, self.H, self.W, self.C)
            nxt = self.next
            if isinstance(nxt, ConvStage) and nxt.layer.k == 1 and not nxt.layer.trainable and not o16:
                probe = ops.LayerPlan(ops.DS_CONV_FWD, self.eng.arith, self.eng.plan_options(), B, self.H, self.W, self.C,
                                      nxt.layer.cout, 1, 1, self.C, nxt.layer.cout, DS_EPI_STATS)
                self.raw = probe.norm_supported()
            self.rs = (p.layer.rstd, p.layer.shift)
        if self.raw:
            self.out = self.zmax
        else:
            self.out = torch.empty(B, self.H, self.W, self.C, device=dev, dtype=torch.bfloat16 if o16 else torch.float32)
        self.apply_segs = None
        self.dout = torch.empty(B, self.H, self.W, self.C, device=dev)
        self.argmax = torch.empty(B, self.H, self.W, self.C, dtype=torch.uint8, device=dev)
        self._own_amax = self.eng.new_amax()
        targets = ()
        if isinstance(p, ConvStage) and self.k == 3 and self.stride == 2:
            if self.eng.bwd_sums or inside:
                targets = ((p.layer, 0),)
        elif self.eng.bwd_sums and isinstance(p, MixedStage):
            targets = p.concat_layers()
        for layer, off in targets:
            layer.sums_from_pool(0, self, off)

    @property
    def out_amax(self):
        if self.prev.fused_into_pool:
            return self._own_amax
        return self.prev.out_amax

    def forward(self):
        p = self.prev
        if self.zmax is not None:
            if not self.raw:
                if self.apply_segs is None:
                    am = self._own_amax if self.track_amax else None
                    self.apply_segs = make_segments([(0, self.C, self.out.data_ptr(), self.C, ops.act_dtype(self.out), ops._p(am))])
                ops.bn_apply_relu(p.layer.z, self.B * self.H * self.W, self.C, self.rs[0], self.rs[1], self.apply_segs)
            return
        if p.fused_into_pool and p.pool_applies_bn():
            ops.maxpool_bn_relu_fwd(p.layer.z, p.layer.rstd, p.layer.shift, self.out, self.argmax, self.B, p.H, p.W, p.C,
                                    self.k, self.stride, amax=self._own_amax if self.track_amax else None)
        elif p.zcat:
            ops.maxpool_bn_relu_fwd(p.out, p.rs_cat[0], p.rs_cat[1], self.out, self.argmax, self.B, p.H, p.W, p.C,
                                    self.k, self.stride)
        else:
            if p.out.dtype != self.out.dtype:
                raise RuntimeError("%s: input and output storage differ (fuse_bn_pool switched after alloc?)" % self.name)
            ops.maxpool_fwd(p.out, self.out, self.argmax, self.B, p.H, p.W, p.C, self.k, self.stride, "SAME")

    def backward(self, need_dx):
        p = self.prev
        if p.fused_into_pool and self.stride == 2:
            return
        if need_dx:
            ops.maxpool_bwd(self.dout, self.argmax, p.dout, False, self.B, p.H, p.W, p.C, self.k, self.stride, "SAME")


class MixedStage(Stage):

    def __init__(self, eng, name, prev, b0, b1, b2, b3, trainable, beta_bucket):
        self.eng, self.name, self.prev = eng, name, prev
        (b1a, b1b), (b2a, b2b) = b1, b2
        self.b = (b0, b1a, b1b, b2a, b2b, b3)
        self.H, self.W, self.C = prev.H, prev.W, b0 + b1b + b2b + b3
        cin = prev.C
        pre = "InceptionV1/%s/" % name
        b2b_scope = "Conv2d_0a_3x3" if name == "Mixed_5b" else "Conv2d_0b_3x3"
        nf = b0 + b1a + b2a
        self.fused = ConvBN(eng, [(pre + "Branch_0/Conv2d_0a_1x1", 0, b0),
                                  (pre + "Branch_1/Conv2d_0a_1x1", b0, b0 + b1a),
                                  (pre + "Branch_2/Conv2d_0a_1x1", b0 + b1a, nf)],
                            1, 1, cin, nf, self.H, self.W, trainable, beta_bucket)
        self.c1 = ConvBN(eng, [(pre + "Branch_1/Conv2d_0b_3x3", 0, b1b)], 3, 1, b1a, b1b, self.H, self.W, trainable,
                         beta_bucket)
        self.c2 = ConvBN(eng, [(pre + "Branch_2/" + b2b_scope, 0, b2b)], 3, 1, b2a, b2b, self.H, self.W, trainable,
                         beta_bucket)
        self.c3 = ConvBN(eng, [(pre + "Branch_3/Conv2d_0b_1x1", 0, b3)], 1, 1, cin, b3, self.H, self.W, trainable,
                         beta_bucket)
        self.layers = [self.fused, self.c1, self.c2, self.c3]
        self.c2.slot, self.c3.slot = 1, 2
        self.ev = None

    def concat_layers(self):
        b0, _, b1b, _, b2b, _ = self.b
        return ((self.fused, 0), (self.c1, b0), (self.c2, b0 + b1b), (self.c3, b0 + b1b + b2b))

    def alloc(self, B):
        eng, dev = self.eng, self.eng.device
        b0, b1a, b1b, b2a, b2b, b3 = self.b
        cin, Ct = self.prev.C, self.C
        self.B = B
        M = B * self.H * self.W
        for l in self.layers:
            l.alloc(B)
        out16 = eng.act16 and self.name not in ("Mixed_5b", "Mixed_5c")
        r16 = eng.act16 and self.name != "Mixed_5c"
        a16 = lambda f: torch.bfloat16 if f else torch.float32
        self.out = torch.empty(B, self.H, self.W, Ct, device=dev, dtype=a16(out16))
        self.dout = torch.empty(B, self.H, self.W, Ct, device=dev)
        self.r1 = torch.empty(M, b1a, device=dev, dtype=a16(r16))
        self.r2 = torch.empty(M, b2a, device=dev, dtype=a16(r16))
        self.dr1 = torch.empty(M, b1a, device=dev)
        self.dr2 = torch.empty(M, b2a, device=dev)
        self.dpooled = torch.empty(M, cin, device=dev)
        self.argmax = torch.empty(M, cin, dtype=torch.uint8, device=dev)
        self.fuse_b3 = bool(eng.fuse_branch3 and not self.c3.trainable and eng.dtype == "f32" and not eng.act16
                            and self.c3.fwd.enable_pool3(self.argmax))
        if self.fuse_b3:
            eng.need_stats(self.c3.fwd.partials * 2 * b3)
        self.pooled = None if self.fuse_b3 else torch.empty(M, cin, device=dev, dtype=self.prev.out.dtype)
        o, do = self.out.data_ptr(), self.dout.data_ptr()
        nf = b0 + b1a + b2a
        es, dt_o, dt_r = self.out.element_size(), ops.act_dtype(self.out), ops.act_dtype(self.r1)
        self.out_amax, self.r1_amax, self.r2_amax = eng.new_amax(), eng.new_amax(), eng.new_amax()
        am_o, am_1, am_2 = ops._p(self.out_amax), ops._p(self.r1_amax), ops._p(self.r2_amax)
        self.seg_f = make_segments([(0, b0, o, Ct, dt_o, am_o), (b0, b0 + b1a, self.r1.data_ptr(), b1a, dt_r, am_1),
                                    (b0 + b1a, nf, self.r2.data_ptr(), b2a, dt_r, am_2)])
        self.seg_1, self.seg_2, self.seg_3 = (make_segments([(0, layer.cout, o + es * off, Ct, dt_o, am_o)])
                                              for layer, off in self.concat_layers()[1:])
        self.fused.set_dy_parts([(0, b0, do, Ct), (b0, b0 + b1a, self.dr1.data_ptr(), b1a),
                                 (b0 + b1a, nf, self.dr2.data_ptr(), b2a)])
        for layer, off in self.concat_layers()[1:]:
            layer.set_dy_parts([(0, layer.cout, do + 4 * off, Ct)])
        self.zcat = self._zcat_ok(B)
        self.rs_cat = None
        self.batch_bn = 0
        self._infer_close = None
        self._fz_close = None
        if self.zcat:
            self.rs_cat = torch.empty(2, Ct, device=dev)
            self.rs_cat[0].fill_(1.0)
            self.rs_cat[1].zero_()
            self.mean_cat = torch.zeros(Ct, device=dev)
            self.coef_cat = torch.empty(2, Ct - b0, device=dev)
            zc = self.out.view(M, Ct)
            for layer, off in self.concat_layers()[1:]:
                n = layer.cout
# ... 60 lines not shown
        eng = self.eng
        if not (eng.branch_streams and eng.side):
            for chain in ((branch3, tail, branch2) if head is None else (head, tail, branch2, branch3)):
                chain()
            return
        main = torch.cuda.current_stream()
        one = eng.one_side_stream
        s3 = eng.side[1]
        if self.ev is None:
            self.ev = [torch.cuda.Event() for _ in range(4)]
        e_in, e_f, e_2, e_3 = self.ev
        e_in.record(main)
        with torch.cuda.stream(s3):
            s3.wait_event(e_in)
            branch3()
            if not one:
                e_3.record(s3)
        if head is not None:
            head()
        if one == 2:
            e_2.record(s3)
            branch2()
        else:
            s2 = s3 if one else eng.side[0]
            if head is not None:
                e_f.record(main)
            with torch.cuda.stream(s2):
                if head is not None:
                    s2.wait_event(e_f)
                elif not one:
                    s2.wait_event(e_in)
                branch2()
                e_2.record(s2)
        tail()
        main.wait_event(e_2)
        if not one:
            main.wait_event(e_3)

    def _zcat_ok(self, B):
        eng = self.eng
        nxt = self.next
        if not (eng.zcat and eng.dtype == "f32" and not eng.act16 and not eng.train_all):
            return False
        if any(l.trainable for l in self.layers):
            return False
        if isinstance(nxt, PoolStage):
            return True
        if isinstance(nxt, MixedStage) and not any(l.trainable for l in nxt.layers):
            nf = nxt.b[0] + nxt.b[1] + nxt.b[3]
            probe = ops.LayerPlan(ops.DS_CONV_FWD, eng.arith, eng.plan_options(), B, self.H, self.W, self.C, nf, 1, 1, self.C,
                                  nf, DS_EPI_STATS)
            return probe.norm_supported()
        return False

    def _pool_fwd(self):
        p = self.prev
        if self.fuse_b3:
            return
        if p.zcat:
            ops.maxpool_bn_relu_fwd(p.out, p.rs_cat[0], p.rs_cat[1], self.pooled, self.argmax, self.B, p.H, p.W, p.C, 3, 1)
        else:
            ops.maxpool_fwd(p.out, self.pooled, self.argmax, self.B, p.H, p.W, p.C, 3, 1, "SAME")

    def _batch_forward(self):
        eng = self.eng
        return bool((self.batch_bn & 1) and eng.batch_stats and not eng.sync_bn
                    and all(l.fin is None for l in (self.c1, self.c2, self.c3)))

    def _finalize_closing(self):
        eng = self.eng
        jobs = self._fin_jobs.get(eng.update_moving)
        if jobs is None:
            jobs = ops.BnFinalizeJobs([(l.stats_buf, l.fwd.partials, l.M, l.cout, l.beta, l.mean, l.mean, l.rstd, l.shift,
                                        l.mm if eng.update_moving else None, l.mv if eng.update_moving else None)
                                       for l in (self.c1, self.c2, self.c3)])
            self._fin_jobs[eng.update_moving] = jobs
        jobs.run(BN_EPS, BN_DECAY)

    def _batch_backward(self, need_dx):
        eng = self.eng
        return bool((self.batch_bn & 2) and need_dx and not eng.sync_bn
                    and all(l.dz16 is None and not l.bnb and l.dgrad.family != ops.DS_FAM_FP8D for l in (self.c1, self.c2, self.c3)))

    def _bn_backward_closing(self):
        b0 = self.b[0]
        Ct, Cb = self.C, self.C - b0
        M = self.B * self.H * self.W
        layers = (self.c1, self.c2, self.c3)
        if self._close_plan is None:
            sg = ops.SumSegments()
            sg.nseg = 3
            off = 0
            for i, l in enumerate(layers):
                ls = l._sum_plan()
                assert ls.nseg == 1
                sg.c_begin[i], sg.c_end[i] = off, off + l.cout
                sg.P[i], sg.kind[i], sg.s[i], sg.q[i] = ls.P[0], ls.kind[0], ls.s[0], ls.q[0]
                off += l.cout
            assert off == Cb
            dy = make_segments([(0, Cb, self.dout.data_ptr() + 4 * b0, Ct)])
            self._close_plan = (sg, dy, self.out.view(M, Ct)[:, b0:])
        sg, dy, z = self._close_plan
        for l in layers:
            l._run_reduce_jobs()
        if self.eng.fuse_fin_apply:
            ops.bn_bwd_finalize_apply(sg, M, Cb, None, None, self.coef_cat, z, dy, self.mean_cat[b0:], self.rs_cat[0, b0:],
                                      self.rs_cat[1, b0:], z, self.fa_ticket, ldz=Ct, betas=[l.beta for l in layers],
                                      dbetas=[l.gbeta for l in layers])
        else:
            ops.bn_bwd_finalize_multi(sg, M, Cb, [l.beta for l in layers], [l.gbeta for l in layers], self.coef_cat)
            ops.bn_bwd_apply(z, dy, M, Cb, self.mean_cat[b0:], self.rs_cat[0, b0:], self.rs_cat[1, b0:], self.coef_cat, z, ldz=Ct)
        for l in layers:
            l._dz_amax_live = False

    def forward(self):
        p = self.prev
        b0, b1a, b1b, b2a, b2b, b3 = self.b
        x = ops._p(p.out)
        dx_, dr_ = ops.act_dtype(p.out), ops.act_dtype(self.r1)
        ax_, a1_, a2_ = p.out_amax, self.r1_amax, self.r2_amax
        defer = self._batch_forward()

        def branch3():
            self._pool_fwd()
            self.c3.forward(x if self.fuse_b3 else ops._p(self.pooled), p.C, self.seg_3, dx_, ax_, defer)

        self._fork_join(lambda: self.fused.forward(x, p.C, self.seg_f, dx_, ax_),
                        lambda: self.c1.forward(ops._p(self.r1), b1a, self.seg_1, dr_, a1_, defer),
                        lambda: self.c2.forward(ops._p(self.r2), b2a, self.seg_2, dr_, a2_, defer), branch3)
        if defer:
            self._finalize_closing()

    def backward(self, need_dx):
        p = self.prev
        b0, b1a, b1b, b2a, b2b, b3 = self.b
        x = ops._p(p.out)
        eng = self.eng
        pool_first = need_dx and self.pool_first
        keep = self.fused.dgrad.d.flags & ops.DS_EPI_BNSUMS
        self.fused.dgrad.d.flags = (ops.DS_EPI_ACCUM if pool_first else 0) | keep

        infer = eng.infer_bwd
        batched = self._batch_backward(need_dx) and not infer
        if batched:
            self._bn_backward_closing()
        if infer and self.zcat:
            M, Ct = self.B * self.H * self.W, self.C
            if self._infer_close is None:
                self._infer_close = (make_segments([(0, Ct - b0, self.dout.data_ptr() + 4 * b0, Ct)]), self.out.view(M, Ct)[:, b0:])
            dy, z = self._infer_close
            if eng.frozen_step and self.c1.gbeta is not None:
                if self._fz_close is None:
                    P = ops.bn_infer_bwd_partials(M, Ct - b0)
                    self._fz_close = torch.empty((Ct - b0) * P, device=eng.device)
                    off = 0
                    for l in (self.c1, self.c2, self.c3):
                        l.fz_job = (self._fz_close.data_ptr() + 4 * off * P, P)
                        off += l.cout
                ops.bn_infer_bwd_apply_sums(z, dy, M, Ct - b0, self.rs_cat[0, b0:], self.rs_cat[1, b0:], z, self._fz_close, ldz=Ct)
            else:
                ops.bn_infer_bwd_apply(z, dy, M, Ct - b0, self.rs_cat[0, b0:], self.rs_cat[1, b0:], z, ldz=Ct)

        def closing(layer, x_ptr, ldx, dx_ptr, ndx):
            if eng.frozen_step:
                layer.backward_frozen(x_ptr, ldx, dx_ptr, ndx, apply=not self.zcat)
            elif infer:
                layer.backward_infer(dx_ptr, apply=not self.zcat)
            elif batched:
                layer._run_dgrad(dx_ptr)
            else:
                layer.backward(x_ptr, ldx, dx_ptr, ndx)

        def branch3():
            closing(self.c3, None if self.fuse_b3 else ops._p(self.pooled), p.C, ops._p(self.dpooled), need_dx)
            if pool_first:
                ops.maxpool_bwd(self.dpooled, self.argmax, p.dout, False, self.B, p.H, p.W, p.C, 3, 1, "SAME")
            elif need_dx and self.split_dout and infer:
                ops.maxpool_bwd(self.dpooled, self.argmax, p.dout2, False, self.B, p.H, p.W, p.C, 3, 1, "SAME")
            elif need_dx and self.split_dout:
                ops.maxpool3_bwd_sums(self.dpooled, self.argmax, p.dout2, False, p.out, self.B, p.H, p.W, p.C, self.pool_sums)

        self._fork_join(None, lambda: closing(self.c1, ops._p(self.r1), b1a, ops._p(self.dr1), True),
                        lambda: closing(self.c2, ops._p(self.r2), b2a, ops._p(self.dr2), True), branch3)
        if infer:
            if eng.frozen_step:
                self.fused.backward_frozen(x, p.C, ops._p(p.dout) if need_dx else None, need_dx)
            else:
                self.fused.backward_infer(ops._p(p.dout))
            if need_dx and not pool_first and not self.split_dout:
                ops.maxpool_bwd(self.dpooled, self.argmax, p.dout, True, self.B, p.H, p.W, p.C, 3, 1, "SAME")
            return
        self.fused.backward(x, p.C, ops._p(p.dout) if need_dx else None, need_dx)
        if need_dx and self.split_dout:
            ops.bn_bwd_reduce(p.out, self._dgrad_sum_segs, self.B * p.H * p.W, p.C, eng.zeros, eng.ones, eng.zeros, self.dgrad_sums,
                              ldz=p.C)
        if need_dx and not pool_first and not self.split_dout:
            if self.pool_sums is not None:
                ops.maxpool3_bwd_sums(self.dpooled, self.argmax, p.dout, True, p.out, self.B, p.H, p.W, p.C, self.pool_sums)
            else:
                ops.maxpool_bwd(self.dpooled, self.argmax, p.dout, True, self.B, p.H, p.W, p.C, 3, 1, "SAME")


class InceptionV1Engine:

    def __init__(self, store, num_classes, image_size=224, dropout_keep_prob=0.8, trainable_bn_beta=True,
                 device="cuda", train_all=False, dtype="f32"):
        self.store, self.num_classes, self.keep = store, num_classes, dropout_keep_prob
        assert dtype in ("f32", "bf16", "fp8")
        self.dtype = dtype
        self.conv_dtype = ops.DS_DTYPE_F32 if dtype == "f32" else ops.DS_DTYPE_BF16
        self.trainable_bn_beta = trainable_bn_beta
        self.train_all = train_all
        self.device = torch.device(device)
        self.update_moving = True
        self.training = True
        self.reducer = None
        self.sync_bn = False
        self.sync_world = 1
        self.sync_group = None
        self.seed_dev = None
        self.side_mode = None
        self.one_side_stream = 1
        self.pool_first = True
        self.act16 = dtype in ("bf16", "fp8") and not train_all
        self.wgrad_side = True
        self.side_w = None
        self.wgrad_stream = None
        self.bwd_sums = True
        self.stem_direct = True
        self.stem_pool = _lib.tuning_env("DS_STEM_POOL", "1") != "0"
        self.branch_streams = True
        self.side = None
        self.fp8_everywhere = _lib.tuning_env("DS_FP8_EVERYWHERE", "0") == "1"
        self.fp8_wide_rule = _lib.tuning_env("DS_FP8_RULE", "0") == "1"
        self.bf16_direct = True
        self.wino16 = _lib.tuning_env("DS_WINO16", "1") != "0"
        self.winograd = True
        self.mul3 = _lib.tuning_env("DS_MUL3", "0") == "1"
        self.bnb_on_load = int(_lib.tuning_env("DS_BNB", "1"))
        self.zcat = _lib.tuning_env("DS_ZCAT", "1") != "0"
        self.fuse_finalize = _lib.tuning_env("DS_FUSE_FIN", "0") == "1"
        self.fuse_fin_apply = _lib.tuning_env("DS_FIN_APPLY", "0") == "1"
        e = _lib.tuning_env("DS_BATCH_BN")
        self.batch_bn = int(e) if e else None
        self.pool_sums = _lib.tuning_env("DS_POOL_SUMS", "1") != "0"
        self.split_dout = _lib.tuning_env("DS_SPLIT_DOUT", "0") == "1"
        self.z16 = _lib.tuning_env("DS_Z16", "1") != "0"
        self.dpooled16 = _lib.tuning_env("DS_DPOOLED16", "0") == "1"
        self.stem_sums_from_dgrad = _lib.tuning_env("DS_STEM_SUMS", "1") != "0"
        self.dz16 = int(_lib.tuning_env("DS_DZ16", "2"))
        self.fuse_branch3 = _lib.tuning_env("DS_FUSE_B3", "1") != "0"
        self.winograd4 = _lib.tuning_env("DS_WINO4", "1") != "0"
        self.splitk = _lib.tuning_env("DS_SPLITK", "1") != "0"
        e = _lib.tuning_env("DS_TEXT_GATE")
        self.text_gate = int(e) if e else None
        self.text_gate_event = None
        self.weights_version = 0
        self.fused_infer = False
        self.fused_request = False
        self._fused_key = None
        self._fused_targets = {}
        self._fused_jobs = None
        self.input_grad = False
        self.infer_bwd = False
        self.frozen_step = False
        self._frozen_prep = None
        self._frozen_jobs = {}
        self._input_grad_training = True
        self._pivots = None
        self._restore_pivots = None
        self._stats_n = self._bwdp_n = self._ws_bytes = 0
        self.B = None
        self.alloc_gen = 0
        self.input = InputStage(self, image_size)
        self.stages = []
        prev = self.input
        for item in TOPOLOGY:
            kind, name = item[0], item[1]
            tr = train_all or name in TRAINABLE_ENDPOINTS
            bucket = 1 if tr else 2
            if kind == "conv":
                st = ConvStage(self, name, prev, item[2], item[3], item[4], tr, bucket)
            elif kind == "maxpool":
                st = PoolStage(self, name, prev, item[2], item[3])
            else:
                st = MixedStage(self, name, prev, item[2], item[3], item[4], item[5], tr, bucket)
            self.stages.append(st)
            prev = st
        self.last = prev
        for a, b in zip(self.stages[:-1], self.stages[1:]):
            a.next = b
        self.fuse_bn_pool = True
        assert self.last.H == 7 and self.last.W == 7, "AvgPool_0a_7x7 + SpatialSqueeze need a 7x7 map (224x224 input)"
        self.feat = self.last.C
        lg = "InceptionV1/Logits/Conv2d_0c_1x1"
        store.declare(lg + "/weights", (1, 1, self.feat, num_classes), True, l2=True, bucket=1)
        store.declare(lg + "/biases", (num_classes,), True, bucket=1)
        self.lg = lg
        self.layers = [l for s in self.stages for l in s.layers]

    @property
    def batch_stats(self):
        return bool(self.training and not self.frozen_step)

    @property
    def arith(self):
        if self.dtype == "f32":
            return ops.DS_ARITH_F32X3 if self.mul3 else ops.DS_ARITH_F32
        return ops.DS_ARITH_BF16 if self.dtype == "bf16" else ops.DS_ARITH_FP8

    def plan_options(self):
        o = 0
        if not self.winograd:
            o |= ops.DS_PLAN_NO_WINO
        if not self.winograd4:
            o |= ops.DS_PLAN_NO_WINO4
        if not self.stem_direct:
            o |= ops.DS_PLAN_NO_STEM_DIRECT
        if not self.bf16_direct:
            o |= ops.DS_PLAN_NO_BF16_DIRECT
        if self.act16:
            o |= ops.DS_PLAN_ACT16
        if self.fp8_everywhere:
# ... 322 lines not shown
```

### tumblr_emotions_amd/ops.py

```python
import ctypes as C
import os

import torch

from . import _lib
from ._lib import (ConvDesc, Segments, SumSegments, DS_EPI_ACCUM, DS_EPI_BIAS, DS_EPI_BNSUMS, DS_EPI_MASK, DS_EPI_RELU,
                   DS_EPI_STATS, DS_EPI_BN_RELU,
                   DS_DTYPE_BF16, DS_DTYPE_F32, DS_FP8_E4M3, DS_FP8_E5M2, DS_CONV_FWD, DS_CONV_DGRAD, DS_ARITH_F32, DS_ARITH_BF16,
                   DS_ARITH_FP8, DS_ARITH_F32X3, DS_FAM_IGEMM, DS_FAM_WINO2, DS_FAM_WINO4, DS_FAM_STEM, DS_FAM_BF16D, DS_FAM_FP8D,
                   DS_FAM_F32X3, DS_FAM_WINO4H, DS_FAM_STEM_POOL, DS_FAM_STEM_DGRAD, DS_PLAN_STEM_POOL, DS_PLAN_NO_SPLITK, DS_PLAN_NO_WINO4H, DS_PLAN_NO_WINO, DS_PLAN_NO_WINO4, DS_PLAN_NO_STEM_DIRECT, DS_PLAN_NO_BF16_DIRECT, DS_PLAN_ACT16,
                   DS_PLAN_PACKED_RGB, DS_PLAN_FP8_EVERYWHERE, DS_PLAN_FP8_WIDE_RULE)


_raw_stream = getattr(torch._C, "_cuda_getCurrentRawStream", None)


def _stream():
    if _raw_stream is not None:
        return C.c_void_p(_raw_stream(torch.cuda.current_device()))
    return C.c_void_p(torch.cuda.current_stream().cuda_stream)


def _p(t):
    if t is None:
# ... 547 lines not shown

def bn_bwd_partials(M, C_):
    return _lib.load().ds_bn_bwd_partials(M, C_)


def bn_bwd_reduce(z, segs, M, C_, mean, rstd, shift, partials, ldz=None, z_dtype=DS_DTYPE_F32):
    ptr = lambda t: t if isinstance(t, C.c_void_p) else _p(t)
    if not isinstance(z, C.c_void_p):
        z_dtype = act_dtype(z)
    _lib.check(_lib.load().ds_bn_bwd_reduce(ptr(z), C_ if ldz is None else ldz, z_dtype, C.byref(segs), M, C_, ptr(mean),
                                            ptr(rstd), ptr(shift), ptr(partials), _stream()), "ds_bn_bwd_reduce")


def bn_bwd_finalize_segs(sum_segs, M, C_, beta, dbeta, coef):
    _lib.check(_lib.load().ds_bn_bwd_finalize_segs(C.byref(sum_segs), M, C_, _p(beta), _p(dbeta), _p(coef), _stream()),
               "ds_bn_bwd_finalize_segs")


class BnFinalizeJobs:

    def __init__(self, jobs):
        self.n = len(jobs)
        self.arr = (_lib.BnFinalizeJob * self.n)()
        self._keep = jobs
        for a, (stats, P, count, C_, beta, pivot, mean, rstd, shift, mm, mv) in zip(self.arr, jobs):
            a.stats, a.P, a.C, a.count = stats.data_ptr(), P, C_, count
            a.beta, a.pivot = beta.data_ptr(), (pivot.data_ptr() if pivot is not None else None)
            a.mean, a.rstd, a.shift = mean.data_ptr(), rstd.data_ptr(), shift.data_ptr()
            a.moving_mean = mm.data_ptr() if mm is not None else None
            a.moving_var = mv.data_ptr() if mv is not None else None

    def run(self, eps, decay):
        _lib.check(_lib.load().ds_bn_finalize_multi(C.cast(self.arr, C.c_void_p), self.n, eps, decay, _stream()),
                   "ds_bn_finalize_multi")


def bn_bwd_finalize_multi(sum_segs, M, C_, betas, dbetas, coef):
    n = sum_segs.nseg
    b = (C.c_void_p * 4)(*[t.data_ptr() for t in betas[:n]])
    d = (C.c_void_p * 4)(*[(t.data_ptr() if t is not None else None) for t in dbetas[:n]])
    _lib.check(_lib.load().ds_bn_bwd_finalize_multi(C.byref(sum_segs), M, C_, C.cast(b, C.c_void_p), C.cast(d, C.c_void_p),
                                                    _p(coef), _stream()), "ds_bn_bwd_finalize_multi")


def bn_finalize_apply_relu(stats, P, count, C_, beta, eps, decay, mean, rstd, shift, mm, mv, pivot, z, M, segs, ticket):
    _lib.check(_lib.load().ds_bn_finalize_apply_relu(_p(stats), P, count, C_, _p(beta), _p(pivot), eps, decay, _p(mean), _p(rstd),
                                                     _p(shift), _p(mm), _p(mv), _p(z), M, C.byref(segs), _p(ticket), _stream()),
               "ds_bn_finalize_apply_relu")


def bn_bwd_finalize_apply(sum_segs, M, C_, beta, dbeta, coef, z, segs, mean, rstd, shift, dz, ticket, amax=None, ldz=0,
                          betas=None, dbetas=None):
    bv = dv = None
    if betas is not None:
        n = sum_segs.nseg
        bv = C.cast((C.c_void_p * 4)(*[t.data_ptr() for t in betas[:n]]), C.c_void_p)
        dv = C.cast((C.c_void_p * 4)(*[(t.data_ptr() if t is not None else None) for t in dbetas[:n]]), C.c_void_p)
    out16 = dz.dtype == torch.bfloat16
    _lib.check(_lib.load().ds_bn_bwd_finalize_apply(C.byref(sum_segs), _p(beta), _p(dbeta), bv, dv, _p(coef), _p(z), ldz or C_,
                                                    C.byref(segs), M, C_, _p(mean), _p(rstd), _p(shift), _p(dz),
                                                    DS_DTYPE_BF16 if out16 else DS_DTYPE_F32, dz.stride(0) if out16 else 0,
                                                    _p(amax), _p(ticket), _stream()), "ds_bn_bwd_finalize_apply")


def bn_bwd_finalize(partials, P, M, C_, dbeta, coef):
    _lib.check(_lib.load().ds_bn_bwd_finalize(_p(partials), P, M, C_, _p(dbeta), _p(coef), _stream()),
               "ds_bn_bwd_finalize")


def bn_bwd_apply(z, segs, M, C_, mean, rstd, shift, coef, dz, amax=None, ldz=0):
    if z.dtype == torch.bfloat16:
        assert dz.dtype == torch.bfloat16
        _lib.check(_lib.load().ds_bn_bwd_apply_z16(_p(z), ldz or C_, C.byref(segs), M, C_, _p(mean), _p(rstd), _p(shift),
                                                   _p(coef), _p(dz), dz.stride(0), _p(amax), _stream()), "ds_bn_bwd_apply_z16")
        return
    if dz.dtype == torch.bfloat16:
        _lib.check(_lib.load().ds_bn_bwd_apply_bf16(_p(z), ldz or C_, C.byref(segs), M, C_, _p(mean), _p(rstd), _p(shift),
                                                    _p(coef), _p(dz), dz.stride(0), _p(amax), _stream()), "ds_bn_bwd_apply_bf16")
        return
    _lib.check(_lib.load().ds_bn_bwd_apply(_p(z), ldz or C_, C.byref(segs), M, C_, _p(mean), _p(rstd), _p(shift), _p(coef),
                                           _p(dz), _p(amax), _stream()), "ds_bn_bwd_apply")


def bn_infer_bwd_apply(z, segs, M, C_, rstd, shift, dz, ldz=0):
    ptr = lambda t: t if isinstance(t, C.c_void_p) else _p(t)
    _lib.check(_lib.load().ds_bn_infer_bwd_apply(ptr(z), ldz or C_, C.byref(segs), M, C_, ptr(rstd), ptr(shift), ptr(dz),
                                                 _stream()), "ds_bn_infer_bwd_apply")


def bn_infer_bwd_partials(M, C_):
    return _lib.load().ds_bn_infer_bwd_partials(M, C_)


def bn_infer_bwd_apply_sums(z, segs, M, C_, rstd, shift, dz, partials, ldz=0):
    ptr = lambda t: t if isinstance(t, C.c_void_p) else _p(t)
    _lib.check(_lib.load().ds_bn_infer_bwd_apply_sums(ptr(z), ldz or C_, C.byref(segs), M, C_, ptr(rstd), ptr(shift), ptr(dz),
                                                      ptr(partials), _stream()), "ds_bn_infer_bwd_apply_sums")


class BnSumJobs:

    def __init__(self, jobs):
        self.n = len(jobs)
        self.arr = (_lib.BnSumJob * self.n)()
        self._keep = jobs
        for a, (partials, P, C_, dbeta) in zip(self.arr, jobs):
            a.partials = partials if isinstance(partials, int) else partials.data_ptr()
            a.P, a.C, a.dbeta = P, C_, dbeta.data_ptr()

    def run(self):
        _lib.check(_lib.load().ds_bn_dbeta_reduce_multi(C.cast(self.arr, C.c_void_p), self.n, _stream()),
                   "ds_bn_dbeta_reduce_multi")


def maxpool_fwd(x, y, argmax, N, H, W, C_, k, stride, mode="SAME"):
    if mode == "SAME":
        OH, pt = same_pad(H, k, stride)
        OW, pl = same_pad(W, k, stride)
    else:
        OH, OW, pt, pl = (H - k) // stride + 1, (W - k) // stride + 1, 0, 0
    assert x.dtype == y.dtype
    _lib.check(_lib.load().ds_maxpool_fwd(_p(x), _p(y), _p(argmax), N, H, W, C_, k, stride, pt, pl, OH, OW,
                                          act_dtype(x), _stream()), "ds_maxpool_fwd")
    return OH, OW


def maxpool_bn_relu_fwd(z, rstd, shift, y, argmax, N, H, W, C_, k, stride, amax=None):
    OH, pt = same_pad(H, k, stride)
    OW, pl = same_pad(W, k, stride)
    _lib.check(_lib.load().ds_maxpool_bn_relu_fwd(_p(z), _p(rstd), _p(shift), _p(y), _p(argmax), N, H, W, C_, k, stride,
                                                  pt, pl, OH, OW, act_dtype(y), _p(amax), _stream()),
               "ds_maxpool_bn_relu_fwd")
    return OH, OW


def bn_pool_bwd_partials(N, H, W, C_):
    OH, _ = same_pad(H, 3, 2)
    OW, _ = same_pad(W, 3, 2)
    return _lib.load().ds_bn_pool_bwd_partials(N, OH, OW, C_)


def bn_pool_bwd_reduce(z, dpool, argmax, N, H, W, C_, mean, rstd, shift, partials):
    OH, pt = same_pad(H, 3, 2)
    OW, pl = same_pad(W, 3, 2)
    _lib.check(_lib.load().ds_bn_pool_bwd_reduce(_p(z), _p(dpool), _p(argmax), N, H, W, C_, pt, pl, OH, OW, _p(mean),
                                                 _p(rstd), _p(shift), _p(partials), _stream()), "ds_bn_pool_bwd_reduce")


def bn_pool_bwd_apply(z, dpool, argmax, N, H, W, C_, mean, rstd, shift, coef, dz):
    OH, pt = same_pad(H, 3, 2)
    OW, pl = same_pad(W, 3, 2)
    _lib.check(_lib.load().ds_bn_pool_bwd_apply(_p(z), _p(dpool), _p(argmax), N, H, W, C_, pt, pl, OH, OW, _p(mean),
                                                _p(rstd), _p(shift), _p(coef), _p(dz), _stream()), "ds_bn_pool_bwd_apply")


def bn_pool_infer_bwd_apply(z, dpool, argmax, N, H, W, C_, rstd, shift, dz):
    OH, pt = same_pad(H, 3, 2)
    OW, pl = same_pad(W, 3, 2)
    _lib.check(_lib.load().ds_bn_pool_infer_bwd_apply(_p(z), _p(dpool), _p(argmax), N, H, W, C_, pt, pl, OH, OW, _p(rstd),
                                                      _p(shift), _p(dz), _stream()), "ds_bn_pool_infer_bwd_apply")


def bn_pool_infer_bwd_apply_sums(z, dpool, argmax, N, H, W, C_, rstd, shift, dz, partials):
    OH, pt = same_pad(H, 3, 2)
    OW, pl = same_pad(W, 3, 2)
    _lib.check(_lib.load().ds_bn_pool_infer_bwd_apply_sums(_p(z), _p(dpool), _p(argmax), N, H, W, C_, pt, pl, OH, OW, _p(rstd),
                                                           _p(shift), _p(dz), _p(partials), _stream()),
               "ds_bn_pool_infer_bwd_apply_sums")


def maxpool_bwd(dy, argmax, dx, accumulate, N, H, W, C_, k, stride, mode="SAME"):
    if dy.dtype == torch.bfloat16:
        assert k == 3 and stride == 1 and mode == "SAME"
        _lib.check(_lib.load().ds_maxpool3_bwd_dy16(_p(dy), _p(argmax), _p(dx), int(accumulate), None, DS_DTYPE_F32, N, H, W, C_,
                                                    None, _stream()), "ds_maxpool3_bwd_dy16")
        return
    if mode == "SAME":
        OH, pt = same_pad(H, k, stride)
        OW, pl = same_pad(W, k, stride)
    else:
        OH, OW, pt, pl = (H - k) // stride + 1, (W - k) // stride + 1, 0, 0
    _lib.check(_lib.load().ds_maxpool_bwd(_p(dy), _p(argmax), _p(dx), int(accumulate), N, H, W, C_, k, stride, pt,
                                          pl, OH, OW, _stream()), "ds_maxpool_bwd")


def maxpool3_bwd_sums_partials(N, W, C_):
    return _lib.load().ds_maxpool3_bwd_sums_partials(N, W, C_)


def maxpool3_bwd_sums(dy, argmax, dx, accumulate, y, N, H, W, C_, partials):
    if dy.dtype == torch.bfloat16:
        _lib.check(_lib.load().ds_maxpool3_bwd_dy16(_p(dy), _p(argmax), _p(dx), int(accumulate), _p(y), act_dtype(y), N, H, W, C_,
                                                    _p(partials), _stream()), "ds_maxpool3_bwd_dy16")
        return
    _lib.check(_lib.load().ds_maxpool3_bwd_sums(_p(dy), _p(argmax), _p(dx), int(accumulate), _p(y), act_dtype(y), N, H, W, C_,
                                                _p(partials), _stream()), "ds_maxpool3_bwd_sums")


def avgpool_dropout_fwd(x, N, HW, C_, keep, seed, mask_in, mask_out, out, seed_dev=None):
    _lib.check(_lib.load().ds_avgpool_dropout_fwd(_p(x), N, HW, C_, keep, seed, _p(seed_dev), _p(mask_in),
                                                  _p(mask_out), _p(out), _stream()), "ds_avgpool_dropout_fwd")


def avgpool_dropout_bwd(dout, mask, N, HW, C_, keep, dx):
    _lib.check(_lib.load().ds_avgpool_dropout_bwd(_p(dout), _p(mask), N, HW, C_, keep, _p(dx), _stream()),
               "ds_avgpool_dropout_bwd")


def gather_rows(table, ids, out, B, T, D, time_major=True):
    _lib.check(_lib.load().ds_gather_rows(_p(table), _p(ids), _p(out), B, T, D, table.shape[0], int(time_major),
                                          _stream()), "ds_gather_rows")


def embedding_grad(dx, ids, dtable, B, T, D, time_major=True):
    _lib.check(_lib.load().ds_embedding_grad(_p(dx), _p(ids), _p(dtable), B, T, D, dtable.shape[0], int(time_major),
                                             _stream()), "ds_embedding_grad")


def token_dot(dx, x, seq_len, out, B, T, D):
    _lib.check(_lib.load().ds_token_dot(_p(dx), _p(x), _p(seq_len), _p(out), B, T, D, _stream()), "ds_token_dot")


def lstm_cell_fwd(gates, c_prev, h_prev, seq_len, t, B, H, forget_bias, c_out, h_out, rec_slabs=None, nslabs=0,
                  slab_stride=0):
    _lib.check(_lib.load().ds_lstm_cell_fwd(_p(gates), _p(rec_slabs), nslabs, slab_stride, _p(c_prev), _p(h_prev),
                                            _p(seq_len), t, B, H, forget_bias, _p(c_out), _p(h_out), _stream()),
               "ds_lstm_cell_fwd")


def lstm_cell_bwd(acts, c_t, c_prev, dh, dc, seq_len, t, B, H, dgates, dc_prev, dh_carry, dh_slabs=None, nslabs=0,
                  slab_stride=0):
    _lib.check(_lib.load().ds_lstm_cell_bwd(_p(acts), _p(c_t), _p(c_prev), _p(dh), _p(dh_slabs), nslabs, slab_stride,
                                            _p(dc), _p(seq_len), t, B, H, _p(dgates), _p(dc_prev), _p(dh_carry),
                                            _stream()), "ds_lstm_cell_bwd")


# ... 538 lines not shown
```

Before: 19400 samples/s.

## Fuse maxpool backward into BN backward apply for mixed stages before stride-2 pools

For Inception mixed stages followed by a stride-2 max pool, the BN backward apply now reads the pooled gradient and argmax directly and scatters per-pixel gradients inside the apply kernel. This skips the separate maxpool_bwd pass that wrote the full-resolution dout. The kernel is column-range aware, so the batched closing BN and the fused first branch each get their slice, and a new column-slice apply handles the remaining branches. It is on by default via DS_POOL_APPLY but gated by many conditions; when those fail, the old maxpool_bwd path still runs. Risks are wrong gradients if the geometry or branch assumptions are violated.

```diff
diff --git a/include/ds_kernels.h b/include/ds_kernels.h
--- a/include/ds_kernels.h
+++ b/include/ds_kernels.h
@@ -309,6 +309,9 @@
                              int32_t lddz, float *amax, uint32_t *ticket, void *stream);
 int ds_bn_bwd_apply(const float *z, int32_t ldz, const ds_segments *dy, int64_t M, int32_t C, const float *mean,
                     const float *rstd, const float *shift, const float *coef, float *dz, float *amax, void *stream);
+int ds_bn_bwd_apply_cols(const float *z, int32_t ldz, const ds_segments *dy, int64_t M, int32_t ncols, const float *mean,
+                         const float *rstd, const float *shift, const float *coef_g, const float *coef_gx, float *dz,
+                         void *stream);
 int ds_bn_infer_bwd_apply(const float *z, int32_t ldz, const ds_segments *dy, int64_t M, int32_t C, const float *rstd,
                           const float *shift, float *dz, void *stream);
 int ds_bn_infer_bwd_partials(int64_t M, int32_t C);
@@ -341,6 +344,10 @@
 int ds_bn_pool_bwd_apply(const float *z, const float *dpool, const uint8_t *argmax, int32_t N, int32_t H, int32_t W,
                          int32_t C, int32_t pad_t, int32_t pad_l, int32_t OH, int32_t OW, const float *mean,
                          const float *rstd, const float *shift, const float *coef, float *dz, void *stream);
+int ds_bn_pool_bwd_apply_cols(const float *z, int32_t ldz, float *dz, int32_t lddz, const float *dpool, const uint8_t *argmax,
+                              int32_t Cp, int32_t c0, int32_t N, int32_t H, int32_t W, int32_t pad_t, int32_t pad_l, int32_t OH,
+                              int32_t OW, int32_t ncols, const float *mean, const float *rstd, const float *shift,
+                              const float *coef_g, const float *coef_gx, int32_t k, void *stream);
 int ds_bn_pool_infer_bwd_apply(const float *z, const float *dpool, const uint8_t *argmax, int32_t N, int32_t H, int32_t W,
                                int32_t C, int32_t pad_t, int32_t pad_l, int32_t OH, int32_t OW, const float *rstd,
                                const float *shift, float *dz, void *stream);
diff --git a/tumblr_emotions_amd/_lib.py b/tumblr_emotions_amd/_lib.py
--- a/tumblr_emotions_amd/_lib.py
+++ b/tumblr_emotions_amd/_lib.py
@@ -218,6 +218,7 @@
     "ds_bn_finalize_apply_relu": (C.c_int, [_P, _i32, _i64, _i32, _P, _P, _f32, _f32, _P, _P, _P, _P, _P, _P, _i64, _SG, _P, _P]),
     "ds_bn_bwd_finalize_apply": (C.c_int, [_SS, _P, _P, _P, _P, _P, _P, _i32, _SG, _i64, _i32, _P, _P, _P, _P, _i32, _i32, _P, _P, _P]),
     "ds_bn_bwd_apply": (C.c_int, [_P, _i32, _SG, _i64, _i32, _P, _P, _P, _P, _P, _P, _P]),
+    "ds_bn_bwd_apply_cols": (C.c_int, [_P, _i32, _SG, _i64, _i32, _P, _P, _P, _P, _P, _P, _P]),
     "ds_bn_infer_bwd_apply": (C.c_int, [_P, _i32, _SG, _i64, _i32, _P, _P, _P, _P]),
     "ds_bn_infer_bwd_partials": (C.c_int, [_i64, _i32]),
     "ds_bn_infer_bwd_apply_sums": (C.c_int, [_P, _i32, _SG, _i64, _i32, _P, _P, _P, _P, _P]),
@@ -228,6 +229,7 @@
     "ds_bn_pool_bwd_partials": (C.c_int, [_i32, _i32, _i32, _i32]),
     "ds_bn_pool_bwd_reduce": (C.c_int, [_P, _P, _P] + [_i32] * 8 + [_P, _P, _P, _P, _P]),
     "ds_bn_pool_bwd_apply": (C.c_int, [_P, _P, _P] + [_i32] * 8 + [_P, _P, _P, _P, _P, _P]),
+    "ds_bn_pool_bwd_apply_cols": (C.c_int, [_P, _i32, _P, _i32, _P, _P] + [_i32] * 10 + [_P, _P, _P, _P, _P, _i32, _P]),
     "ds_bn_pool_infer_bwd_apply": (C.c_int, [_P, _P, _P] + [_i32] * 8 + [_P, _P, _P, _P]),
     "ds_bn_pool_infer_bwd_apply_sums": (C.c_int, [_P, _P, _P] + [_i32] * 8 + [_P, _P, _P, _P, _P]),
     "ds_maxpool_bwd": (C.c_int, [_P, _P, _P] + [_i32] * 11 + [_P]),
diff --git a/tumblr_emotions_amd/csrc/bn.hip b/tumblr_emotions_amd/csrc/bn.hip
--- a/tumblr_emotions_amd/csrc/bn.hip
+++ b/tumblr_emotions_amd/csrc/bn.hip
@@ -425,13 +425,14 @@
 template <bool OUT16, bool COH = false, bool ADD2 = false, bool Z16 = false>
 __device__ __forceinline__ void bwd_apply_body(int bid, const float *z, int ldz, const SegDev &dy, int64_t M, int C,
                                                const float *mean, const float *rstd, const float *shift,
-                                               const float *coef, float *dz, float *amax, int drow, int lddz) {
+                                               const float *coef, float *dz, float *amax, int drow, int lddz,
+                                               const float *coef_gx = nullptr) {
     const int C4 = C >> 2;
     const int t0 = bid * 256 + threadIdx.x;
     const int row0 = t0 / C4, c = (t0 - row0 * C4) * 4;
     const float4 r4 = *reinterpret_cast<const float4 *>(rstd + c), s4 = *reinterpret_cast<const float4 *>(shift + c);
     const float4 m4 = *reinterpret_cast<const float4 *>(mean + c);
-    const float4 k14 = ld_res4<COH>(coef + c), k24 = ld_res4<COH>(coef + C + c);
+    const float4 k14 = ld_res4<COH>(coef + c), k24 = ld_res4<COH>((coef_gx ? coef_gx : coef + C) + c);
     const float rr[4] = {r4.x, r4.y, r4.z, r4.w}, ss[4] = {s4.x, s4.y, s4.z, s4.w}, mm[4] = {m4.x, m4.y, m4.z, m4.w};
     const float a1[4] = {k14.x, k14.y, k14.z, k14.w}, a2[4] = {k24.x, k24.y, k24.z, k24.w};
     int sgi = 0;
@@ -491,8 +492,9 @@
 template <bool OUT16, bool ADD2 = false, bool Z16 = false>
 __global__ __launch_bounds__(256) void bn_bwd_apply_kernel(const float *z, int ldz, SegDev dy, int64_t M, int C,
                                                            const float *mean, const float *rstd, const float *shift,
-                                                           const float *coef, float *dz, float *amax, int drow, int lddz) {
-    bwd_apply_body<OUT16, false, ADD2, Z16>((int)blockIdx.x, z, ldz, dy, M, C, mean, rstd, shift, coef, dz, amax, drow, lddz);
+                                                           const float *coef, float *dz, float *amax, int drow, int lddz,
+                                                           const float *coef_gx = nullptr) {
+    bwd_apply_body<OUT16, false, ADD2, Z16>((int)blockIdx.x, z, ldz, dy, M, C, mean, rstd, shift, coef, dz, amax, drow, lddz, coef_gx);
 }
 
 template <bool ADD2>
@@ -962,6 +964,21 @@
         hipLaunchKernelGGL(bn_bwd_apply_kernel<false>, dim3(grid), dim3(256), 0, (hipStream_t)stream, z, ldz, to_dev(dy), M, C, mean, rstd,
                            shift, coef, dz, amax, drow, ldz);
     return ds::check_launch("ds_bn_bwd_apply");
+}
+
+extern "C" int ds_bn_bwd_apply_cols(const float *z, int32_t ldz, const ds_segments *dy, int64_t M, int32_t ncols, const float *mean,
+                                    const float *rstd, const float *shift, const float *coef_g, const float *coef_gx, float *dz,
+                                    void *stream) {
+    DS_REQUIRE(z && mean && rstd && shift && coef_g && coef_gx && dz && M > 0 && ncols > 0 && ncols % 4 == 0 && ldz >= ncols &&
+                   ldz % 4 == 0 && ((((uintptr_t)z) | ((uintptr_t)dz) | ((uintptr_t)coef_g) | ((uintptr_t)coef_gx)) & 15) == 0,
+               "ds_bn_bwd_apply_cols: bad argument (need ncols %% 4 == 0, ldz >= ncols, ldz %% 4 == 0, 16-byte aligned z / dz / coef)");
+    if (int e = check_segments(dy, ncols, "ds_bn_bwd_apply_cols")) return e;
+    DS_REQUIRE(!has_second_addend(dy), "ds_bn_bwd_apply_cols: no second addend");
+    int drow;
+    const int grid = column_grid(M, ncols / 4, &drow);
+    hipLaunchKernelGGL(bn_bwd_apply_kernel<false>, dim3(grid), dim3(256), 0, (hipStream_t)stream, z, ldz, to_dev(dy), M, ncols, mean, rstd,
+                       shift, coef_g, dz, (float *)nullptr, drow, ldz, coef_gx);
+    return ds::check_launch("ds_bn_bwd_apply_cols");
 }
 
 extern "C" int ds_bn_bwd_apply_z16(const void *z16, int32_t ldz, const ds_segments *dy, int64_t M, int32_t C, const float *mean,
diff --git a/tumblr_emotions_amd/csrc/pool.hip b/tumblr_emotions_amd/csrc/pool.hip
--- a/tumblr_emotions_amd/csrc/pool.hip
+++ b/tumblr_emotions_amd/csrc/pool.hip
@@ -711,6 +711,76 @@
     }
 }
 
+template <int K>
+__global__ __launch_bounds__(256) void bn_pool_bwd_apply_cols_kernel(const float *z, int ldz, float *dz, int lddz,
+                                                                     const float *dpool, const uint8_t *am, int Cp, int N,
+                                                                     int H, int W, int pad_t, int pad_l, int OH, int OW,
+                                                                     int ncols, const float *mean, const float *rstd,
+                                                                     const float *shift, const float *coef_g,
+                                                                     const float *coef_gx) {
+    constexpr int E = K == 3 ? 1 : 0;
+    const int C4 = ncols >> 2;
+    const int PH = OH + E, PW = OW + E;
+    const int64_t total = (int64_t)N * PH * PW * C4;
+    for (int64_t i = (int64_t)blockIdx.x * 256 + threadIdx.x; i < total; i += (int64_t)gridDim.x * 256) {
+        const int c = (int)(i % C4) * 4;
+        int64_t r = i / C4;
+        const int q = (int)(r % PW) - E;
+        r /= PW;
+        const int p = (int)(r % PH) - E;
+        const int n = (int)(r / PH);
+        PatchGrad pg;
+        if constexpr (K == 3) {
+            pg = patch_grad(dpool, am, n, p, q, c, Cp, OH, OW);
+        } else {
+            const int64_t o = (((int64_t)n * OH + p) * OW + q) * Cp + c;
+            const unsigned a = *reinterpret_cast<const unsigned *>(am + o);
+            const float4 t = *reinterpret_cast<const float4 *>(dpool + o);
+            const float d[4] = {t.x, t.y, t.z, t.w};
+#pragma unroll
+            for (int y = 0; y < 2; ++y)
+#pragma unroll
+                for (int x = 0; x < 2; ++x)
+#pragma unroll
+                    for (int j = 0; j < 4; ++j) {
+                        pg.g[y][x][j] = 0.f;
+                        if (((a >> (8 * j)) & 0xFFu) == (unsigned)(y * 2 + x)) pg.g[y][x][j] += d[j];
+                    }
+        }
+        const float4 r4 = *reinterpret_cast<const float4 *>(rstd + c);
+        const float4 s4 = *reinterpret_cast<const float4 *>(shift + c);
+        const float4 m4 = *reinterpret_cast<const float4 *>(mean + c);
+        const float4 k1 = *reinterpret_cast<const float4 *>(coef_g + c);
+        const float4 k2 = *reinterpret_cast<const float4 *>(coef_gx + c);
+        const float rr[4] = {r4.x, r4.y, r4.z, r4.w}, ss[4] = {s4.x, s4.y, s4.z, s4.w}, mm[4] = {m4.x, m4.y, m4.z, m4.w};
+        const float a1[4] = {k1.x, k1.y, k1.z, k1.w}, a2[4] = {k2.x, k2.y, k2.z, k2.w};
+        float4 zv[2][2];
+        bool ok[2][2];
+        int64_t pix[2][2];
+#pragma unroll
+        for (int y = 0; y < 2; ++y)
+#pragma unroll
+            for (int x = 0; x < 2; ++x) {
+                const int ih = 2 * p - pad_t + E + y, iw = 2 * q - pad_l + E + x;
+                ok[y][x] = (unsigned)ih < (unsigned)H && (unsigned)iw < (unsigned)W;
+                pix[y][x] = ((int64_t)n * H + ih) * W + iw;
+                zv[y][x] = make_float4(0.f, 0.f, 0.f, 0.f);
+                if (ok[y][x]) zv[y][x] = ds::ld_stream4(z + pix[y][x] * ldz + c);
+            }
+#pragma unroll
+        for (int y = 0; y < 2; ++y)
+#pragma unroll
+            for (int x = 0; x < 2; ++x) {
+                if (!ok[y][x]) continue;
+                const float zz[4] = {zv[y][x].x, zv[y][x].y, zv[y][x].z, zv[y][x].w};
+                float o[4];
+#pragma unroll
+                for (int j = 0; j < 4; ++j) o[j] = ds::bn_bwd_dz(zz[j], pg.g[y][x][j], rr[j], ss[j], mm[j], a1[j], a2[j]);
+                *reinterpret_cast<float4 *>(dz + pix[y][x] * lddz + c) = make_float4(o[0], o[1], o[2], o[3]);
+            }
+    }
+}
+
 __global__ __launch_bounds__(256) void bn_pool_infer_bwd_apply_kernel(const float *z, const float *dpool, const uint8_t *am,
                                                                       int N, int H, int W, int C, int pad_t, int pad_l, int OH,
                                                                       int OW, const float *rstd, const float *shift, float *dz) {
@@ -1009,6 +1079,37 @@
     return ds::check_launch("ds_bn_pool_bwd_apply");
 }
 
+extern "C" int ds_bn_pool_bwd_apply_cols(const float *z, int32_t ldz, float *dz, int32_t lddz, const float *dpool,
+                                         const uint8_t *argmax, int32_t Cp, int32_t c0, int32_t N, int32_t H, int32_t W,
+                                         int32_t pad_t, int32_t pad_l, int32_t OH, int32_t OW, int32_t ncols,
+                                         const float *mean, const float *rstd, const float *shift, const float *coef_g,
+                                         const float *coef_gx, int32_t k, void *stream) {
+    DS_REQUIRE(z && dz && dpool && argmax && mean && rstd && shift && coef_g && coef_gx,
+               "ds_bn_pool_bwd_apply_cols: null pointer");
+    DS_REQUIRE(k == 2 || k == 3, "ds_bn_pool_bwd_apply_cols: kernel size %d (3: 3x3/2, 2: 2x2/2 pools only)", k);
+    DS_REQUIRE(ncols > 0 && ncols % 4 == 0 && c0 >= 0 && c0 % 4 == 0 && Cp % 4 == 0 && ldz % 4 == 0 && lddz % 4 == 0,
+               "ds_bn_pool_bwd_apply_cols: ncols %d, first column %d and the strides %d / %d / %d must be multiples of 4", ncols, c0,
+               ldz, lddz, Cp);
+    DS_REQUIRE(ldz >= ncols && lddz >= ncols && Cp >= c0 + ncols,
+               "ds_bn_pool_bwd_apply_cols: stride smaller than the column range (ldz %d, lddz %d, pool %d < %d + %d)", ldz, lddz, Cp,
+               c0, ncols);
+    DS_REQUIRE(N > 0 && H > 0 && W > 0 && OH > 0 && OW > 0 && pad_t >= 0 && pad_t <= 1 && pad_l >= 0 && pad_l <= 1,
+               "ds_bn_pool_bwd_apply_cols: bad geometry");
+    DS_REQUIRE(H <= 2 * OH && W <= 2 * OW && (k == 3 || (H + pad_t <= 2 * OH && W + pad_l <= 2 * OW)),
+               "ds_bn_pool_bwd_apply_cols: H > 2 OH or W > 2 OW (stride-2 SAME pools only)");
+    DS_REQUIRE(((((uintptr_t)z) | ((uintptr_t)dz) | ((uintptr_t)dpool) | ((uintptr_t)mean) | ((uintptr_t)rstd) | ((uintptr_t)shift) |
+                 ((uintptr_t)coef_g) | ((uintptr_t)coef_gx)) & 15) == 0 && (((uintptr_t)argmax) & 3) == 0,
+               "ds_bn_pool_bwd_apply_cols: 16-byte aligned tensors and vectors, 4-byte aligned winners");
+    const dim3 grid(pool_bwd_grid(N, OH, OW, ncols));
+    if (k == 3)
+        hipLaunchKernelGGL(bn_pool_bwd_apply_cols_kernel<3>, grid, dim3(256), 0, (hipStream_t)stream, z, ldz, dz, lddz, dpool + c0,
+                           argmax + c0, Cp, N, H, W, pad_t, pad_l, OH, OW, ncols, mean, rstd, shift, coef_g, coef_gx);
+    else
+        hipLaunchKernelGGL(bn_pool_bwd_apply_cols_kernel<2>, grid, dim3(256), 0, (hipStream_t)stream, z, ldz, dz, lddz, dpool + c0,
+                           argmax + c0, Cp, N, H, W, pad_t, pad_l, OH, OW, ncols, mean, rstd, shift, coef_g, coef_gx);
+    return ds::check_launch("ds_bn_pool_bwd_apply_cols");
+}
+
 extern "C" int ds_bn_pool_infer_bwd_apply(const float *z, const float *dpool, const uint8_t *argmax, int32_t N, int32_t H,
                                           int32_t W, int32_t C, int32_t pad_t, int32_t pad_l, int32_t OH, int32_t OW,
                                           const float *rstd, const float *shift, float *dz, void *stream) {
diff --git a/tumblr_emotions_amd/engine_image.py b/tumblr_emotions_amd/engine_image.py
--- a/tumblr_emotions_amd/engine_image.py
+++ b/tumblr_emotions_amd/engine_image.py
@@ -184,6 +184,7 @@
         self.dy2 = False
         self.part_pool = [None] * len(parts)
         self._sum_segs = None
+        self._rest_segs = None
 
     def sums_from(self, part, src, src2=None):
         self.part_sums[part], self.part_sums2[part] = src, src2
@@ -515,7 +516,17 @@
         self.dgrad.d.x_dtype = ops.DS_DTYPE_F32
         self.dgrad.run(ops._p(self.z), self.w_ptr, dx_ptr, mask=y, stats=sums, x_amax=ops._p(am))
 
-    def backward(self, x_ptr=None, ldx=0, dx_ptr=None, need_dx=True):
+    def _bwd_apply_pooled(self, pool):
+        b0, nf = self.dy_parts[0][1], self.cout
+        if self._rest_segs is None:
+            self._rest_segs = make_segments([(c0 - b0, c1 - b0, ptr, ld) for (c0, c1, ptr, ld) in self.dy_parts[1:]])
+        ops.bn_pool_bwd_apply_cols(self.z, nf, self.z, nf, pool.dout, pool.argmax, pool.C, 0, self.B, self.OH, self.OW, b0,
+                                   self.mean, self.rstd, self.shift, self.coef[0], self.coef[1], pool.k)
+        zr = self.z[:, b0:]
+        ops.bn_bwd_apply_cols(zr, self._rest_segs, self.M, nf - b0, self.mean[b0:], self.rstd[b0:], self.shift[b0:],
+                              self.coef[0, b0:], self.coef[1, b0:], zr, ldz=nf)
+
+    def backward(self, x_ptr=None, ldx=0, dx_ptr=None, need_dx=True, pool=None):
         eng = self.eng
         M, Cc = self.M, self.cout
         dy_segs = self.dy_segs
@@ -525,6 +536,7 @@
         track = self.dgrad is not None and self.dgrad.family == ops.DS_FAM_FP8D
         dz = self.z if self.dz16 is None else self.dz16
         if eng.fuse_fin_apply and not eng.sync_bn and (need_dx or self.trainable) and not self.bnb and not self.dy2 and not self.z16:
+            assert pool is None
             if from_parts:
                 sg = self._sum_plan()
                 self._run_reduce_jobs()
@@ -550,8 +562,12 @@
             if self.bnb:
                 self._run_dgrad(dx_ptr)
                 return
-            ops.bn_bwd_apply(self.z, dy_segs, M, Cc, self.zmean, self.rstd, self.zshift, self.coef, dz,
-                             amax=self.dz_amax if track else None, ldz=self.ldz)
+            if pool is not None:
+                assert from_parts and not self.bnb and not track and dz is self.z and self.ldz == Cc
+                self._bwd_apply_pooled(pool)
+            else:
+                ops.bn_bwd_apply(self.z, dy_segs, M, Cc, self.zmean, self.rstd, self.zshift, self.coef, dz,
+                                 amax=self.dz_amax if track else None, ldz=self.ldz)
         self._dz_amax_live = track
         if self.trainable:
             self._run_wgrad(x_ptr, ldx)
@@ -569,6 +585,7 @@
     raw = False
     out_amax = None
     fused_into_pool = False
+    pooled_bwd = False
     track_amax = True
 
 
@@ -691,6 +708,11 @@
             targets = p.concat_layers()
         for layer, off in targets:
             layer.sums_from_pool(0, self, off)
+        eng = self.eng
+        p.pooled_bwd = bool(eng.pool_apply and isinstance(p, MixedStage) and targets and self.stride == 2 and self.k in (2, 3)
+                            and eng.dtype == "f32" and not eng.act16 and p.fused.dgrad.family != ops.DS_FAM_FP8D
+                            and p.zcat and (p.batch_bn & 2) and not eng.split_dout and not p.fused.bnb and p.fused.dz16 is None
+                            and not p.fused.z16 and p.b[0] % 4 == 0)
 
     @property
     def out_amax(self):
@@ -722,7 +744,7 @@
         p = self.prev
         if p.fused_into_pool and self.stride == 2:
             return
-        if need_dx:
+        if need_dx and not p.pooled_bwd:
             ops.maxpool_bwd(self.dout, self.argmax, p.dout, False, self.B, p.H, p.W, p.C, self.k, self.stride, "SAME")
 
 
@@ -949,7 +971,7 @@
         return bool((self.batch_bn & 2) and need_dx and not eng.sync_bn
                     and all(l.dz16 is None and not l.bnb and l.dgrad.family != ops.DS_FAM_FP8D for l in (self.c1, self.c2, self.c3)))
 
-    def _bn_backward_closing(self):
+    def _bn_backward_closing(self, from_pool=False):
         b0 = self.b[0]
         Ct, Cb = self.C, self.C - b0
         M = self.B * self.H * self.W
@@ -976,7 +998,12 @@
                                       dbetas=[l.gbeta for l in layers])
         else:
             ops.bn_bwd_finalize_multi(sg, M, Cb, [l.beta for l in layers], [l.gbeta for l in layers], self.coef_cat)
-            ops.bn_bwd_apply(z, dy, M, Cb, self.mean_cat[b0:], self.rs_cat[0, b0:], self.rs_cat[1, b0:], self.coef_cat, z, ldz=Ct)
+            if from_pool:
+                nx = self.next
+                ops.bn_pool_bwd_apply_cols(z, Ct, z, Ct, nx.dout, nx.argmax, Ct, b0, self.B, self.H, self.W, Cb, self.mean_cat[b0:],
+                                           self.rs_cat[0, b0:], self.rs_cat[1, b0:], self.coef_cat[0], self.coef_cat[1], nx.k)
+            else:
+                ops.bn_bwd_apply(z, dy, M, Cb, self.mean_cat[b0:], self.rs_cat[0, b0:], self.rs_cat[1, b0:], self.coef_cat, z, ldz=Ct)
         for l in layers:
             l._dz_amax_live = False
 
@@ -1009,8 +1036,12 @@
 
         infer = eng.infer_bwd
         batched = self._batch_backward(need_dx) and not infer
+        from_pool = self.pooled_bwd and batched and not eng.fuse_fin_apply
+        if self.pooled_bwd and not from_pool:
+            nx = self.next
+            ops.maxpool_bwd(nx.dout, nx.argmax, self.dout, False, self.B, self.H, self.W, self.C, nx.k, nx.stride, "SAME")
         if batched:
-            self._bn_backward_closing()
+            self._bn_backward_closing(from_pool)
         if infer and self.zcat:
             M, Ct = self.B * self.H * self.W, self.C
             if self._infer_close is None:
@@ -1057,7 +1088,7 @@
             if need_dx and not pool_first and not self.split_dout:
                 ops.maxpool_bwd(self.dpooled, self.argmax, p.dout, True, self.B, p.H, p.W, p.C, 3, 1, "SAME")
             return
-        self.fused.backward(x, p.C, ops._p(p.dout) if need_dx else None, need_dx)
+        self.fused.backward(x, p.C, ops._p(p.dout) if need_dx else None, need_dx, pool=self.next if from_pool else None)
         if need_dx and self.split_dout:
             ops.bn_bwd_reduce(p.out, self._dgrad_sum_segs, self.B * p.H * p.W, p.C, eng.zeros, eng.ones, eng.zeros, self.dgrad_sums,
                               ldz=p.C)
@@ -1106,6 +1137,7 @@
         self.mul3 = _lib.tuning_env("DS_MUL3", "0") == "1"
         self.bnb_on_load = int(_lib.tuning_env("DS_BNB", "1"))
         self.zcat = _lib.tuning_env("DS_ZCAT", "1") != "0"
+        self.pool_apply = _lib.tuning_env("DS_POOL_APPLY", "1") != "0"
         self.fuse_finalize = _lib.tuning_env("DS_FUSE_FIN", "0") == "1"
         self.fuse_fin_apply = _lib.tuning_env("DS_FIN_APPLY", "0") == "1"
         e = _lib.tuning_env("DS_BATCH_BN")
diff --git a/tumblr_emotions_amd/ops.py b/tumblr_emotions_amd/ops.py
--- a/tumblr_emotions_amd/ops.py
+++ b/tumblr_emotions_amd/ops.py
@@ -653,6 +653,11 @@
                                            _p(dz), _p(amax), _stream()), "ds_bn_bwd_apply")
 
 
+def bn_bwd_apply_cols(z, segs, M, ncols, mean, rstd, shift, coef_g, coef_gx, dz, ldz):
+    _lib.check(_lib.load().ds_bn_bwd_apply_cols(_p(z), ldz, C.byref(segs), M, ncols, _p(mean), _p(rstd), _p(shift), _p(coef_g),
+                                                _p(coef_gx), _p(dz), _stream()), "ds_bn_bwd_apply_cols")
+
+
 def bn_infer_bwd_apply(z, segs, M, C_, rstd, shift, dz, ldz=0):
     ptr = lambda t: t if isinstance(t, C.c_void_p) else _p(t)
     _lib.check(_lib.load().ds_bn_infer_bwd_apply(ptr(z), ldz or C_, C.byref(segs), M, C_, ptr(rstd), ptr(shift), ptr(dz),
@@ -723,6 +728,14 @@
     OW, pl = same_pad(W, 3, 2)
     _lib.check(_lib.load().ds_bn_pool_bwd_apply(_p(z), _p(dpool), _p(argmax), N, H, W, C_, pt, pl, OH, OW, _p(mean),
                                                 _p(rstd), _p(shift), _p(coef), _p(dz), _stream()), "ds_bn_pool_bwd_apply")
+
+
+def bn_pool_bwd_apply_cols(z, ldz, dz, lddz, dpool, argmax, Cp, c0, N, H, W, ncols, mean, rstd, shift, coef_g, coef_gx, k):
+    OH, pt = same_pad(H, k, 2)
+    OW, pl = same_pad(W, k, 2)
+    _lib.check(_lib.load().ds_bn_pool_bwd_apply_cols(_p(z), ldz, _p(dz), lddz, _p(dpool), _p(argmax), Cp, c0, N, H, W, pt, pl,
+                                                     OH, OW, ncols, _p(mean), _p(rstd), _p(shift), _p(coef_g), _p(coef_gx), k,
+                                                     _stream()), "ds_bn_pool_bwd_apply_cols")
 
 
 def bn_pool_infer_bwd_apply(z, dpool, argmax, N, H, W, C_, rstd, shift, dz):
```

Result: faster. 19770 samples/s, median of 6 (+1.9%).
